# eboigne/PyTV-4D

Hardware: NVIDIA B200
Metric: cp_iter_voxel_updates_per_s (higher is better)
Workload: dtype f32

## Files before the change

__graft_entry__.py:

```python
import os
import subprocess
import sys
from concurrent.futures import ThreadPoolExecutor

ROOT = os.path.dirname(os.path.abspath(__file__))
CSRC = os.path.join(ROOT, "pytv-4d_b200", "csrc")
ARCH = ["-gencode", "arch=compute_100a,code=sm_100a"]
NVCC_FLAGS = ARCH + ["-lineinfo", "-O3", "-std=c++17", "-Xcompiler", "-fPIC"]
SOURCES = ["api.cu", "ops.cu", "tv.cu", "tv_tile.cu", "tv_tile_f64.cu", "tv_tile_norms.cu", "tv_tile_norms_f64.cu", "cp.cu", "cp_extra.cu", "cp_data.cu", "host_api.cu"]
HEADERS = ["core.cuh", "strip_core.cuh", "tile_core.cuh", "tile2_core.cuh", "kernels.cuh", "kernels2.cuh", "kernels_tile.cuh", "tv_path.cuh", "tv_args.cuh", "tmap.cuh", "tv_tile_impl.cuh", "host_common.cuh", os.path.join("..", "..", "include", "pytv_b200.h")]


def source_hash():
    import glob
    import hashlib
    files = sorted(os.path.basename(f) for f in glob.glob(os.path.join(CSRC, "*.cu")) + glob.glob(os.path.join(CSRC, "*.cuh")))
    h = hashlib.sha256()
    for f in files:
        h.update(open(os.path.join(CSRC, f), "rb").read())
    h.update(open(os.path.join(ROOT, "include", "pytv_b200.h"), "rb").read())
    return h.hexdigest()[:16]


def _stale(target, deps):
    if not os.path.exists(target):
        return True
    t = os.path.getmtime(target)
    return any(os.path.getmtime(d) > t for d in deps)


def build(force=False):
    os.makedirs(os.path.join(CSRC, "build"), exist_ok=True)
    hdrs = [os.path.join(CSRC, h) for h in HEADERS]
    src_hash = source_hash()

    def compile_one(src):
        obj = os.path.join(CSRC, "build", src.replace(".cu", ".o"))
        if force or _stale(obj, [os.path.join(CSRC, src)] + hdrs):
            subprocess.run(["nvcc"] + NVCC_FLAGS + ['-DPYTVB_SRC_HASH="%s"' % src_hash, "-c", src, "-o", obj], cwd=CSRC, check=True)
        return obj

    with ThreadPoolExecutor(max_workers=len(SOURCES)) as ex:
        objs = list(ex.map(compile_one, SOURCES))
    lib = os.path.join(CSRC, "libpytv_b200.so")
    if force or _stale(lib, objs):
        subprocess.run(["nvcc"] + ARCH + ["-shared", "-o", lib] + objs, cwd=CSRC, check=True)
    sys.path.insert(0, ROOT)
    if os.path.exists(os.path.join(ROOT, "tests", "emul_helper.py")):
        sys.path.insert(0, os.path.join(ROOT, "tests"))
        import emul_helper
        emul_helper.build_emul(force)
    import pytv_b200
    assert pytv_b200._lib.lib().pytvb_version() == 101
    assert pytv_b200._lib.lib().pytvb_build_id().decode() == src_hash, "the library on disk was not built from these sources"
    return lib


def smoke():
    sys.path.insert(0, ROOT)
    import numpy as np
    import torch
    import pytv_b200 as pytv
    from oracle import tv_oracle as orc

    assert torch.cuda.is_available(), "smoke() needs a CUDA device"
    torch.cuda.set_device(0)
    rs = np.random.RandomState(0)
    x = rs.rand(6, 3, 32, 32).astype(np.float32)
    kw = dict(reg_time=2 ** -5)
    for scheme in ("upwind", "downwind", "central", "hybrid"):
        tv, G = getattr(pytv.tv_GPU, "tv_" + scheme)(x.copy(), **kw)
        tv_o, G_o = orc.tv(x.astype(np.float64), scheme, **kw)
        assert abs(float(tv) - tv_o) <= 1e-5 * tv_o, (scheme, float(tv), tv_o)
        assert np.abs(G - G_o).max() <= 1e-5, (scheme, np.abs(G - G_o).max())
        Dx = getattr(pytv.tv_operators_GPU, "D_" + scheme)(x, **kw)
        assert np.abs(Dx - orc.D(x.astype(np.float64), scheme, **kw)).max() < 1e-5
        DTD = getattr(pytv.tv_operators_GPU, "D_T_" + scheme)(Dx, **kw)
        assert np.abs(DTD - orc.D_T(orc.D(x.astype(np.float64), scheme, **kw), scheme, **kw)).max() < 1e-5
    s = pytv.CPSolver(x, lam=0.1, scheme="hybrid", variant="rof", **kw)
    xo, xb, y = x.astype(np.float64), x.astype(np.float64), np.zeros((6, 8, 3, 32, 32))
    x0 = xo.copy()
    for _ in range(2):
        s.step()
        xo, xb, y, e = orc.cp_rof_step(xo, xb, x0, y, "hybrid", lam=0.1, sigma=0.5, tau=s.tau, theta=1.0, **kw)
    assert abs(s.energy() - e) <= 1e-5 * abs(e), (s.energy(), e)
    assert np.abs(s.result() - xo).max() < 1e-5
    print("smoke ok: TV/D/D_T/CP parity on cuda:0 (%s), %d kernel launches" % (torch.cuda.get_device_name(0), pytv._lib.lib().pytvb_launch_count()))


if __name__ == "__main__":
    build()
    if len(sys.argv) > 1 and sys.argv[1] == "smoke":
        smoke()
```

include/pytv_b200.h:

```cpp
#ifndef PYTV_B200_H
#define PYTV_B200_H

#include <stddef.h>
#include <stdint.h>

#ifdef __cplusplus
extern "C" {
#endif

#define PYTVB_VERSION 101

typedef enum { PYTVB_OK = 0, PYTVB_ERR_ARG = -1, PYTVB_ERR_CUDA = -2 } pytvb_status;

typedef enum { PYTVB_UPWIND = 0, PYTVB_DOWNWIND = 1, PYTVB_CENTRAL = 2, PYTVB_HYBRID = 3 } pytvb_scheme;
typedef enum { PYTVB_F32 = 0, PYTVB_F64 = 1 } pytvb_dtype;

typedef struct pytvb_problem {
    int32_t scheme;
    int32_t dtype;
    int64_t Nz, M, Ni, Nj;
    int64_t z_offset;
    int64_t Nz_global;
    double reg_z_over_reg;
    double reg_time;
    double factor_reg_static;
    const uint8_t* mask_static;
    const void* time_scale;
    const void* time_scale_lo;
    const void* time_scale_hi;
} pytvb_problem;

int pytvb_version(void);
const char* pytvb_build_id(void);
const char* pytvb_last_error(void);
uint64_t pytvb_launch_count(void);

int pytvb_num_components(const pytvb_problem* pb);

size_t pytvb_reduce_workspace_bytes(const pytvb_problem* pb);
size_t pytvb_tv_workspace_bytes(const pytvb_problem* pb);

int pytvb_D(const pytvb_problem* pb, const void* x, void* D, const void* halo_lo, const void* halo_hi, void* stream);

int pytvb_DT(const pytvb_problem* pb, const void* p, void* out, const void* halo_lo, const void* halo_hi, void* stream);

int pytvb_l21(const pytvb_problem* pb, const void* D, int64_t Nd, void* norms_or_null, double* d_sum, void* ws, void* stream);

int pytvb_apply_mask(const pytvb_problem* pb, void* x, const uint8_t* mask, int mask_is_plane, void* stream);

int pytvb_tv(const pytvb_problem* pb, const void* x, void* G, void* norms_or_null, double* d_tv, const void* halo_lo2,
             const void* halo_hi2, void* ws_reduce, void* ws_tv, void* stream);

int pytvb_gd_update(const pytvb_problem* pb, void* x, const void* x0, const void* G, double step, double lam, double* d_fid_or_null, void* ws,
                    void* stream);

int pytvb_tv_value(const pytvb_problem* pb, const void* x, double* d_tv, const void* halo_lo, const void* halo_hi, void* ws, void* stream);

int pytvb_cp_dual(const pytvb_problem* pb, const void* xbar, void* y, double lam, double sigma, double* d_l21_or_null,
                  const void* halo_lo, const void* halo_hi, void* ws, void* stream);

int pytvb_cp_primal_rof(const pytvb_problem* pb, const void* y, void* x, void* xbar, const void* x0, double tau, double theta,
                        double* d_fid_or_null, const void* halo_lo, const void* halo_hi, void* ws, void* stream);

int pytvb_cp_primal_readme(const pytvb_problem* pb, const void* y_tv, void* x, void* y_f, const void* x0, double tau,
                           double sigma_A, double* d_fid_or_null, const void* halo_lo, const void* halo_hi, void* ws,
                           void* stream);

int pytvb_cp_dual_p2p(const pytvb_problem* pb, const void* xbar, void* y, double lam, double sigma, double* d_l21_or_null,
                      const void* halo_lo, const void* halo_hi, void* mirror_prev, void* mirror_next, void* ws, void* stream);
int pytvb_cp_primal_p2p(const pytvb_problem* pb, int variant, const void* y, void* x, void* aux, const void* x0, double tau, double c2,
                        double* d_fid_or_null, const void* halo_lo, const void* halo_hi, void* mirror_prev, void* mirror_next, void* ws,
                        void* stream);

typedef enum { PYTVB_DATA_L2 = 0, PYTVB_DATA_L1 = 1 } pytvb_data_term;
int pytvb_cp_primal_data(const pytvb_problem* pb, int data_term, const void* data_weight, const void* y, void* x, void* xbar,
                         const void* x0, double tau, double theta, double* d_fid_or_null, const void* halo_lo, const void* halo_hi,
                         void* mirror_prev, void* mirror_next, void* ws, void* stream);

int pytvb_cp_dual_f16y(const pytvb_problem* pb, const void* xbar, void* y_half, double lam, double sigma, double* d_l21_or_null,
                       const void* halo_lo, const void* halo_hi, void* ws, void* stream);
int pytvb_cp_primal_rof_f16y(const pytvb_problem* pb, const void* y_half, void* x, void* xbar, const void* x0, double lam, double tau,
                             double theta, double* d_fid_or_null, const void* halo_lo_half, const void* halo_hi_half, void* ws, void* stream);

int pytvb_tv_host(const pytvb_problem* pb_host_mask , const void* x_host, void* G_host,
                  void* norms_host_or_null, double* tv_out);

typedef struct pytvb_cp_solver pytvb_cp_solver;
int pytvb_cp_create(const pytvb_problem* pb_host_mask, double lam, double sigma, double tau, double theta, pytvb_cp_solver** out);
int pytvb_cp_reset_host(pytvb_cp_solver* s, const void* x0_host);
int pytvb_cp_step_host(pytvb_cp_solver* s, const void* x0_host, void* x_host_or_null, double* energy_out);
int pytvb_cp_destroy(pytvb_cp_solver* s);

#ifdef __cplusplus
}
#endif
#endif
```

pytv-4d_b200/_lib.py:

```python
import ctypes
import os

_HERE = os.path.dirname(os.path.abspath(__file__))
LIB_PATH = os.environ.get("PYTVB_LIB_PATH") or os.path.join(_HERE, "csrc", "libpytv_b200.so")

SCHEME_ID = {"upwind": 0, "downwind": 1, "central": 2, "hybrid": 3}
F32, F64 = 0, 1


class Problem(ctypes.Structure):
    _fields_ = [
        ("scheme", ctypes.c_int32),
        ("dtype", ctypes.c_int32),
        ("Nz", ctypes.c_int64),
        ("M", ctypes.c_int64),
        ("Ni", ctypes.c_int64),
        ("Nj", ctypes.c_int64),
        ("z_offset", ctypes.c_int64),
        ("Nz_global", ctypes.c_int64),
        ("reg_z_over_reg", ctypes.c_double),
        ("reg_time", ctypes.c_double),
        ("factor_reg_static", ctypes.c_double),
        ("mask_static", ctypes.c_void_p),
        ("time_scale", ctypes.c_void_p),
        ("time_scale_lo", ctypes.c_void_p),
        ("time_scale_hi", ctypes.c_void_p),
    ]


def make_problem(scheme, dtype_id, shape, reg_z_over_reg=1.0, reg_time=0.0, factor_reg_static=0.0, mask_static_ptr=None,
                 z_offset=0, Nz_global=None, time_scale_ptr=None):
    Nz, M, Ni, Nj = (int(s) for s in shape)
    rz = float(reg_z_over_reg)
    return Problem(SCHEME_ID[scheme] if isinstance(scheme, str) else int(scheme), int(dtype_id), Nz, M, Ni, Nj, int(z_offset),
                   int(Nz if Nz_global is None else Nz_global), rz, float(reg_time), float(factor_reg_static),
                   ctypes.c_void_p(mask_static_ptr) if mask_static_ptr else None,
                   ctypes.c_void_p(time_scale_ptr) if time_scale_ptr else None, None, None)


_VP = ctypes.c_void_p
_PB = ctypes.POINTER(Problem)
_PROTOTYPES = {
    "pytvb_version": (ctypes.c_int, []),
    "pytvb_build_id": (ctypes.c_char_p, []),
    "pytvb_last_error": (ctypes.c_char_p, []),
    "pytvb_launch_count": (ctypes.c_uint64, []),
    "pytvb_num_components": (ctypes.c_int, [_PB]),
    "pytvb_reduce_workspace_bytes": (ctypes.c_size_t, [_PB]),
    "pytvb_tv_workspace_bytes": (ctypes.c_size_t, [_PB]),
    "pytvb_D": (ctypes.c_int, [_PB, _VP, _VP, _VP, _VP, _VP]),
    "pytvb_DT": (ctypes.c_int, [_PB, _VP, _VP, _VP, _VP, _VP]),
    "pytvb_l21": (ctypes.c_int, [_PB, _VP, ctypes.c_int64, _VP, _VP, _VP, _VP]),
    "pytvb_apply_mask": (ctypes.c_int, [_PB, _VP, _VP, ctypes.c_int, _VP]),
    "pytvb_tv": (ctypes.c_int, [_PB, _VP, _VP, _VP, _VP, _VP, _VP, _VP, _VP, _VP]),
    "pytvb_gd_update": (ctypes.c_int, [_PB, _VP, _VP, _VP, ctypes.c_double, ctypes.c_double, _VP, _VP, _VP]),
    "pytvb_tv_value": (ctypes.c_int, [_PB, _VP, _VP, _VP, _VP, _VP, _VP]),
    "pytvb_cp_dual": (ctypes.c_int, [_PB, _VP, _VP, ctypes.c_double, ctypes.c_double, _VP, _VP, _VP, _VP, _VP]),
    "pytvb_cp_primal_rof": (ctypes.c_int, [_PB, _VP, _VP, _VP, _VP, ctypes.c_double, ctypes.c_double, _VP, _VP, _VP, _VP, _VP]),
    "pytvb_cp_primal_readme": (ctypes.c_int, [_PB, _VP, _VP, _VP, _VP, ctypes.c_double, ctypes.c_double, _VP, _VP, _VP, _VP, _VP]),
    "pytvb_cp_dual_p2p": (ctypes.c_int, [_PB, _VP, _VP, ctypes.c_double, ctypes.c_double, _VP, _VP, _VP, _VP, _VP, _VP, _VP]),
    "pytvb_cp_primal_p2p": (ctypes.c_int, [_PB, ctypes.c_int, _VP, _VP, _VP, _VP, ctypes.c_double, ctypes.c_double, _VP, _VP, _VP, _VP, _VP, _VP, _VP]),
    "pytvb_cp_primal_data": (ctypes.c_int, [_PB, ctypes.c_int, _VP, _VP, _VP, _VP, _VP, ctypes.c_double, ctypes.c_double, _VP, _VP, _VP, _VP, _VP, _VP,
                                            _VP]),
    "pytvb_cp_dual_f16y": (ctypes.c_int, [_PB, _VP, _VP, ctypes.c_double, ctypes.c_double, _VP, _VP, _VP, _VP, _VP]),
    "pytvb_cp_primal_rof_f16y": (ctypes.c_int, [_PB, _VP, _VP, _VP, _VP, ctypes.c_double, ctypes.c_double, ctypes.c_double, _VP, _VP, _VP, _VP, _VP]),
    "pytvb_tv_host": (ctypes.c_int, [_PB, _VP, _VP, _VP, ctypes.POINTER(ctypes.c_double)]),
    "pytvb_cp_create": (ctypes.c_int, [_PB, ctypes.c_double, ctypes.c_double, ctypes.c_double, ctypes.c_double, ctypes.POINTER(_VP)]),
    "pytvb_cp_reset_host": (ctypes.c_int, [_VP, _VP]),
    "pytvb_cp_step_host": (ctypes.c_int, [_VP, _VP, _VP, ctypes.POINTER(ctypes.c_double)]),
    "pytvb_cp_destroy": (ctypes.c_int, [_VP]),
}

_lib = None


def lib():
    global _lib
    if _lib is None:
        if not os.path.exists(LIB_PATH):
            raise RuntimeError("pytv_b200: %s has not been built (run __graft_entry__.build()); there is no CPU fallback" % LIB_PATH)
        handle = ctypes.CDLL(LIB_PATH)
        for name, (res, args) in _PROTOTYPES.items():
            fn = getattr(handle, name)
            fn.restype = res
            fn.argtypes = args
        _lib = handle
    return _lib


class PytvError(RuntimeError):
    pass


def check(rc):
    if rc != 0:
        raise PytvError("pytv_b200 call failed (%d): %s" % (rc, lib().pytvb_last_error().decode("utf-8", "replace")))
```

pytv-4d_b200/cp.py:

```python
import ctypes
import os

import numpy as np
import torch

from . import _dev, _lib


DATA_TERMS = {"l2": 0, "l1": 1}


def partition_z(Nz_global, world_size):
    if Nz_global < world_size:
        raise ValueError("cannot split %d planes over %d ranks" % (Nz_global, world_size))
    base, rem = divmod(Nz_global, world_size)
    out, off = [], 0
    for r in range(world_size):
        n = base + (1 if r < rem else 0)
        out.append((off, n))
        off += n
    return out


def operator_norm_sq_bound(scheme, z_on, t_on, reg_z_over_reg, reg_time, factor_reg_static, has_mask_static, max_time_weight=1.0):
    w = 2.0
    if z_on:
        w += reg_z_over_reg
    if t_on:
        w += reg_time * (max(1.0, factor_reg_static) if has_mask_static else 1.0) * max(1.0, float(max_time_weight))
    return w if scheme == "central" else 4.0 * w


class CudaOps:

    def __init__(self):
        self.lib = _lib.lib()

    def cp_dual(self, pb, xbar, y, lam, sigma, d_l21, lo, hi, ws):
        if y.dtype == torch.float16:
            _lib.check(self.lib.pytvb_cp_dual_f16y(ctypes.byref(pb), _dev.ptr(xbar), _dev.ptr(y), lam, sigma, _dev.ptr(d_l21), _dev.ptr(lo),
                                                   _dev.ptr(hi), _dev.ptr(ws), _dev.stream_ptr()))
            return
        _lib.check(self.lib.pytvb_cp_dual(ctypes.byref(pb), _dev.ptr(xbar), _dev.ptr(y), lam, sigma, _dev.ptr(d_l21), _dev.ptr(lo), _dev.ptr(hi),
                                          _dev.ptr(ws), _dev.stream_ptr()))

    def cp_primal(self, variant, pb, y, x, aux, x0, tau, c2, d_fid, lo, hi, ws, lam=None):
        if y.dtype == torch.float16:
            _lib.check(self.lib.pytvb_cp_primal_rof_f16y(ctypes.byref(pb), _dev.ptr(y), _dev.ptr(x), _dev.ptr(aux), _dev.ptr(x0), lam, tau, c2,
                                                         _dev.ptr(d_fid), _dev.ptr(lo), _dev.ptr(hi), _dev.ptr(ws), _dev.stream_ptr()))
            return
        fn = self.lib.pytvb_cp_primal_rof if variant == "rof" else self.lib.pytvb_cp_primal_readme
        _lib.check(fn(ctypes.byref(pb), _dev.ptr(y), _dev.ptr(x), _dev.ptr(aux), _dev.ptr(x0), tau, c2, _dev.ptr(d_fid), _dev.ptr(lo), _dev.ptr(hi),
                      _dev.ptr(ws), _dev.stream_ptr()))

    def cp_primal_data(self, pb, data_term, w, y, x, xbar, x0, tau, theta, d_fid, lo, hi, mirror_prev, mirror_next, ws):
        _lib.check(self.lib.pytvb_cp_primal_data(ctypes.byref(pb), DATA_TERMS[data_term], _dev.ptr(w), _dev.ptr(y), _dev.ptr(x), _dev.ptr(xbar),
                                                 _dev.ptr(x0), tau, theta, _dev.ptr(d_fid), _dev.ptr(lo), _dev.ptr(hi), mirror_prev, mirror_next,
                                                 _dev.ptr(ws), _dev.stream_ptr()))

    def cp_dual_p2p(self, pb, xbar, y, lam, sigma, d_l21, lo, hi, mirror_prev, mirror_next, ws):
        _lib.check(self.lib.pytvb_cp_dual_p2p(ctypes.byref(pb), _dev.ptr(xbar), _dev.ptr(y), lam, sigma, _dev.ptr(d_l21), _dev.ptr(lo), _dev.ptr(hi),
                                              mirror_prev, mirror_next, _dev.ptr(ws), _dev.stream_ptr()))

    def cp_primal_p2p(self, variant, pb, y, x, aux, x0, tau, c2, d_fid, lo, hi, mirror_prev, mirror_next, ws):
        _lib.check(self.lib.pytvb_cp_primal_p2p(ctypes.byref(pb), 0 if variant == "rof" else 1, _dev.ptr(y), _dev.ptr(x), _dev.ptr(aux), _dev.ptr(x0),
                                                tau, c2, _dev.ptr(d_fid), _dev.ptr(lo), _dev.ptr(hi), mirror_prev, mirror_next, _dev.ptr(ws),
                                                _dev.stream_ptr()))

    def workspace(self, pb, device):
        return _dev.reduce_workspace(pb, device)

    def tv_value(self, pb, x, d_tv, lo, hi, ws):
        _lib.check(self.lib.pytvb_tv_value(ctypes.byref(pb), _dev.ptr(x), _dev.ptr(d_tv), _dev.ptr(lo), _dev.ptr(hi), _dev.ptr(ws), _dev.stream_ptr()))

    def adjoint(self, pb, y, out, lo, hi):
        _lib.check(self.lib.pytvb_DT(ctypes.byref(pb), _dev.ptr(y), _dev.ptr(out), _dev.ptr(lo), _dev.ptr(hi), _dev.stream_ptr()))


class HaloExchange:

    def __init__(self, group=None, reduce_group=None):
        import torch.distributed as dist
        self.dist = dist
        self.group = group
        self._reduce_group = reduce_group
        self.rank = dist.get_rank(group)
        self.world = dist.get_world_size(group)
        self.prev = self.rank - 1 if self.rank > 0 else None
        self.next = self.rank + 1 if self.rank < self.world - 1 else None

    def _global(self, r):
        return r if self.group is None else self.dist.get_global_rank(self.group, r)

    def exchange(self, to_prev, to_next, from_prev, from_next):
        self.finish(self.start_exchange(to_prev, to_next, from_prev, from_next))

    def finish(self, reqs):
        for req in reqs or ():
            req.wait()

    def start_exchange(self, to_prev, to_next, from_prev, from_next):
        ops = []
        P2P = self.dist.P2POp
        if self.prev is not None:
            if to_prev is not None:
                ops.append(P2P(self.dist.isend, to_prev, self._global(self.prev), self.group))
            if from_prev is not None:
                ops.append(P2P(self.dist.irecv, from_prev, self._global(self.prev), self.group))
        if self.next is not None:
            if to_next is not None:
                ops.append(P2P(self.dist.isend, to_next, self._global(self.next), self.group))
            if from_next is not None:
                ops.append(P2P(self.dist.irecv, from_next, self._global(self.next), self.group))
        return self.dist.batch_isend_irecv(ops) if ops else []

    def allreduce_sum(self, t):
        self.dist.all_reduce(t, op=self.dist.ReduceOp.SUM, group=self.group)
        return t

    def allreduce_sum_async(self, t):
        g = self._reduce_group if self._reduce_group is not None else self.group
        return self.dist.all_reduce(t, op=self.dist.ReduceOp.SUM, group=g, async_op=True)

    def make_reduce_group(self):
        if self._reduce_group is None and self.group is None:
            self._reduce_group = self.dist.new_group(ranks=list(range(self.dist.get_world_size())))


def neighbour_handshake(hdl, prev, nxt, timeout_ms, sync="auto"):
    if sync == "barrier" or not hasattr(hdl, "put_signal"):
        hdl.barrier(channel=0, timeout_ms=timeout_ms)
        return
    if nxt is not None:
        hdl.put_signal(nxt, channel=1, timeout_ms=timeout_ms)
    if prev is not None:
        hdl.put_signal(prev, channel=2, timeout_ms=timeout_ms)
    if prev is not None:
        hdl.wait_signal(prev, channel=1, timeout_ms=timeout_ms)
    if nxt is not None:
        hdl.wait_signal(nxt, channel=2, timeout_ms=timeout_ms)


class PeerHalos:
    IMG_LO, IMG_HI, FLD_LO, FLD_HI = 0, 1, 2, 3

    def __init__(self, halo, plane, dtype, device):
        import torch.distributed._symmetric_memory as symm
        group = halo.group if halo.group is not None else halo.dist.group.WORLD
        self.buf = symm.empty((4,) + tuple(plane), dtype=dtype, device=device)
        self.hdl = symm.rendezvous(self.buf, group)
        self.buf.zero_()
        self.plane_bytes = self.buf[0].numel() * self.buf.element_size()
        self.timeout_ms = int(os.environ.get("PYTVB_P2P_TIMEOUT_MS", "60000"))
        self.sync = os.environ.get("PYTVB_P2P_SYNC", "auto")
        self.prev, self.next = halo.prev, halo.next
        self.hdl.barrier(channel=0, timeout_ms=self.timeout_ms)

    def local(self, slot):
        return self.buf[slot]

    def peer(self, rank, slot):
        return None if rank is None else int(self.hdl.buffer_ptrs[rank]) + slot * self.plane_bytes

    def barrier(self):
        neighbour_handshake(self.hdl, self.prev, self.next, self.timeout_ms, self.sync)


class CPSolver:

    def __init__(self, x0, lam, scheme="hybrid", variant="rof", sigma=0.5, tau=None, theta=1.0, sigma_A=1.0, reg_z_over_reg=1.0,
                 reg_time=0.0, mask_static=False, factor_reg_static=0, distributed=False, group=None, z_offset=None, Nz_global=None,
                 ops=None, track_energy=True, dual_dtype=None, time_weight=None, comm=None, reduce_group=None, data_term="l2", data_weight=None):
        if scheme not in _dev.SCHEMES:
            raise ValueError("unknown scheme %r" % (scheme,))
        if variant not in ("rof", "readme"):
            raise ValueError("variant must be 'rof' or 'readme'")
        if data_term not in DATA_TERMS:
            raise ValueError("data_term must be 'l2' or 'l1'")
        self.ops = ops if ops is not None else CudaOps()
        self.scheme, self.variant = scheme, variant
        self.lam, self.sigma, self.theta, self.sigma_A = float(lam), float(sigma), float(theta), float(sigma_A)
        self.track_energy = track_energy
        shape = _dev.image_shape(x0)
        if ops is None:
            self.x0, _ = _dev.to_device(x0)
            if self.x0.data_ptr() == (x0.data_ptr() if isinstance(x0, torch.Tensor) else 0):
                self.x0 = self.x0.clone()
        else:
            self.x0 = torch.as_tensor(np.ascontiguousarray(x0)).clone() if not isinstance(x0, torch.Tensor) else x0.clone().contiguous()
        dev, dt = self.x0.device, self.x0.dtype
        self.halo = HaloExchange(group, reduce_group) if (distributed or group is not None) else None
        if self.halo is not None and self.halo.world > 1:
            if track_energy:
                self.halo.make_reduce_group()
            if (Nz_global is None) != (z_offset is None):
                raise ValueError("sharded solver: give both z_offset and Nz_global, or neither (they are then derived from the ranks' plane counts)")
            if Nz_global is None:
                counts = torch.zeros(self.halo.world, dtype=torch.int64, device=dev)
                counts[self.halo.rank] = shape[0]
                self.halo.allreduce_sum(counts)
                Nz_global = int(counts.sum().item())
                z_offset = int(counts[: self.halo.rank].sum().item())
        else:
            self.halo = None
        self.z_offset = int(z_offset or 0)
        self.Nz_global = int(Nz_global if Nz_global is not None else shape[0])
        self.shape = shape
        self._ms = None
        if not isinstance(mask_static, bool):
            if ops is None:
                self._ms = _dev.mask_static_to_device(mask_static, shape[2], shape[3])
            else:
                m = mask_static if isinstance(mask_static, torch.Tensor) else torch.as_tensor(np.asarray(mask_static))
                self._ms = (m.reshape(shape[2], shape[3]) != 0).to(torch.uint8).contiguous()
        self._ts = None
        max_tw = 1.0
        if time_weight is not None:
            w = time_weight if isinstance(time_weight, torch.Tensor) else torch.as_tensor(np.asarray(time_weight))
            w = torch.broadcast_to(w.to(dev).to(torch.float64), shape)
            if bool((w < 0).any()):
                raise ValueError("time_weight must be >= 0")
            self._ts = torch.sqrt(w).to(dt).contiguous()
            mx = w.max().reshape(1).clone()
            if self.halo is not None:
                self.halo.dist.all_reduce(mx, op=self.halo.dist.ReduceOp.MAX, group=self.halo.group)
            max_tw = float(mx.item())
        self.data_term = data_term
        self._dw = None
        self._w_min = 1.0
        if data_weight is not None:
            w = data_weight if isinstance(data_weight, torch.Tensor) else torch.as_tensor(np.asarray(data_weight))
            w = torch.broadcast_to(w.to(dev).to(torch.float64), shape)
            if not bool(torch.isfinite(w).all()) or bool((w < 0).any()):
                raise ValueError("data_weight must be finite and >= 0")
            self._dw = w.to(dt).contiguous()
            mn = self._dw.min().double().reshape(1).clone()
            if self.halo is not None:
                self.halo.dist.all_reduce(mn, op=self.halo.dist.ReduceOp.MIN, group=self.halo.group)
            self._w_min = float(mn.item())
        self._data = data_term != "l2" or self._dw is not None
        self.pb = _lib.make_problem(scheme, _lib.F32 if dt == torch.float32 else _lib.F64, shape, float(reg_z_over_reg), float(reg_time),
                                    float(factor_reg_static), self._ms.data_ptr() if self._ms is not None else None, self.z_offset,
                                    self.Nz_global, self._ts.data_ptr() if self._ts is not None else None)
        self.z_on = self.Nz_global > 1 and float(reg_z_over_reg) > 0
        self.t_on = shape[1] > 1 and float(reg_time) > 0
        self.Nd = (4 + 2 * self.z_on + 2 * self.t_on) if scheme == "hybrid" else (2 + self.z_on + self.t_on)
        if tau is None:
            L2 = operator_norm_sq_bound(scheme, self.z_on, self.t_on, float(reg_z_over_reg), float(reg_time), float(factor_reg_static),
                                        self._ms is not None, max_tw)
            tau = 1.0 / (L2 + 1.0)
        self.tau = float(tau)
        self.x = self.x0.clone()
        self.aux = self.x0.clone() if variant == "rof" else torch.zeros_like(self.x0)
        self.dual_dtype = dt if dual_dtype is None else dual_dtype
        if self.dual_dtype != dt:
            if self.dual_dtype != torch.float16 or dt != torch.float32 or variant != "rof":
                raise ValueError("dual_dtype=torch.float16 needs float32 images and variant='rof'")
            if not self.lam > 0:
                raise ValueError("half-precision dual storage needs lam > 0")
        if self._data and (variant != "rof" or self.dual_dtype != dt):
            raise ValueError("data_term='l1' and data_weight need variant='rof' and full-precision duals")
        self.y = torch.zeros((shape[0], self.Nd) + shape[1:], dtype=self.dual_dtype, device=dev)
        self.scal = torch.zeros(6, dtype=torch.float64, device=dev)
        self.overlap = os.environ.get("PYTVB_OVERLAP", "0") == "1"
        self._pending = None
        self._field_req = None
        self._pb_cache = {}
        self.ws = self.ops.workspace(self.pb, dev)
        self.iterations = 0
        self._img_lo = self._img_hi = self._fld_lo = self._fld_hi = None
        self._peer = None
        if comm is None:
            comm = os.environ.get("PYTVB_COMM", "auto")
        if comm not in ("auto", "nccl", "p2p"):
            raise ValueError("comm must be 'auto', 'nccl' or 'p2p'")
        if self.halo is not None and self.z_on:
            plane = (shape[1], shape[2], shape[3])
            interior_lo, interior_hi = self.halo.prev is not None, self.halo.next is not None
            need_img_lo, need_img_hi = scheme != "upwind", scheme != "downwind"
            need_fld_lo, need_fld_hi = scheme != "downwind", scheme != "upwind"
            p2p_ok = (ops is None and self.dual_dtype == dt and not self.overlap
                      and str(self.halo.dist.get_backend(self.halo.group)).lower() == "nccl")
            if comm == "p2p" and not p2p_ok:
                raise ValueError("comm='p2p' needs the CUDA executor over an NCCL group, the blocking schedule and full-precision duals")
            if comm != "nccl" and p2p_ok:
                try:
                    self._peer = PeerHalos(self.halo, plane, dt, dev)
                except Exception as exc:
                    if comm == "p2p":
                        raise
                    self._peer_error = repr(exc)
                if comm == "auto":
                    ok = torch.tensor([1 if self._peer is not None else 0], dtype=torch.int32, device=dev)
                    self.halo.dist.all_reduce(ok, op=self.halo.dist.ReduceOp.MIN, group=self.halo.group)
                    if int(ok.item()) == 0:
                        self._peer = None
            if self._peer is not None:
                mk = lambda d=dt, slot=0: self._peer.local(slot)
            else:
                mk = lambda d=dt, slot=0: torch.empty(plane, dtype=d, device=dev)
            self._img_lo = mk(slot=0) if (interior_lo and need_img_lo) else None
            self._img_hi = mk(slot=1) if (interior_hi and need_img_hi) else None
            self._fld_lo = mk(self.dual_dtype, 2) if (interior_lo and need_fld_lo) else None
            self._fld_hi = mk(self.dual_dtype, 3) if (interior_hi and need_fld_hi) else None
            if self._peer is not None:
                P, h = self._peer, self.halo
                self._mir_A = (P.peer(h.prev, P.FLD_HI) if need_fld_hi else None, P.peer(h.next, P.FLD_LO) if need_fld_lo else None)
                self._mir_B = (P.peer(h.prev, P.IMG_HI) if need_img_hi else None, P.peer(h.next, P.IMG_LO) if need_img_lo else None)
        self._zf = 4 if scheme == "hybrid" else 2
        self._zb = 5 if scheme == "hybrid" else 2

    def _dual_input(self):
        return self.aux if self.variant == "rof" else self.x

    def _image_planes(self):
        src = self._dual_input()
        return (src[0] if self.scheme != "downwind" else None, src[-1] if self.scheme != "upwind" else None)

    def _start_image_exchange(self):
        return self.halo.start_exchange(*self._image_planes(), self._img_lo, self._img_hi)

    def _start_field_exchange(self):
        to_prev = self.y[0, self._zb] if self.scheme != "upwind" else None
        to_next = self.y[-1, self._zf] if self.scheme != "downwind" else None
        return self.halo.start_exchange(to_prev, to_next, self._fld_lo, self._fld_hi)

    def _sub_problem(self, a, b):
        key = (a, b)
        pb = self._pb_cache.get(key)
        if pb is None:
            pb = _lib.Problem.from_buffer_copy(self.pb)
            pb.Nz = b - a
            pb.z_offset = self.z_offset + a
            if self._ts is not None:
                pb.time_scale = self._ts[a].data_ptr()
            self._pb_cache[key] = pb
        return pb

    def _dual_range(self, a, b, slot):
        if b <= a:
            return
        u = self._dual_input()
        Nz = self.shape[0]
        lo = u[a - 1] if a > 0 else self._img_lo
        hi = u[b] if b < Nz else self._img_hi
        d = self.scal[slot:slot + 1] if self.track_energy else None
        self.ops.cp_dual(self._sub_problem(a, b), u[a:b], self.y[a:b], self.lam, self.sigma, d, lo, hi, self.ws)

    def _primal_range(self, a, b, slot):
        if b <= a:
            return
        Nz = self.shape[0]
        lo = self.y[a - 1, self._zf] if a > 0 else self._fld_lo
        hi = self.y[b, self._zb] if b < Nz else self._fld_hi
        d = self.scal[3 + slot:4 + slot] if self.track_energy else None
        if self._data:
            self.ops.cp_primal_data(self._sub_problem(a, b), self.data_term, self._dw[a:b] if self._dw is not None else None, self.y[a:b], self.x[a:b],
                                    self.aux[a:b], self.x0[a:b], self.tau, self.theta, d, lo, hi, None, None, self.ws)
            return
        c2 = self.theta if self.variant == "rof" else self.sigma_A
        if self.y.dtype == torch.float16:
            self.ops.cp_primal(self.variant, self._sub_problem(a, b), self.y[a:b], self.x[a:b], self.aux[a:b], self.x0[a:b], self.tau, c2, d, lo, hi,
                               self.ws, lam=self.lam)
        else:
            self.ops.cp_primal(self.variant, self._sub_problem(a, b), self.y[a:b], self.x[a:b], self.aux[a:b], self.x0[a:b], self.tau, c2, d, lo,
                               hi, self.ws)

    def _split(self):
        return self.halo is not None and self.z_on and self.overlap and self.shape[0] >= 2

    def _pass_A(self):
        Nz = self.shape[0]
        if self.halo is None or not self.z_on:
            self._dual_range(0, Nz, 0)
            return
        if self._peer is None:
            if self._pending is None:
                self._pending = self._start_image_exchange()
            self.halo.finish(self._pending)
            self._pending = None
        if self.track_energy:
            self.scal[0:3].zero_()
        if self._peer is not None:
            if self._pending is None:
                self.halo.exchange(*self._image_planes(), self._img_lo, self._img_hi)
                self._peer.barrier()
            self._pending = ()
            d = self.scal[0:1] if self.track_energy else None
            self.ops.cp_dual_p2p(self.pb, self._dual_input(), self.y, self.lam, self.sigma, d, self._img_lo, self._img_hi, self._mir_A[0],
                                 self._mir_A[1], self.ws)
            self._peer.barrier()
            self._field_req = ()
            return
        if not self._split():
            self._dual_range(0, Nz, 0)
            self._field_req = self._start_field_exchange()
            return
        self._dual_range(0, 1, 0)
        self._dual_range(Nz - 1, Nz, 1)
        self._field_req = self._start_field_exchange()
        self._dual_range(1, Nz - 1, 2)

    def _pass_B(self):
        Nz = self.shape[0]
        if self.halo is None or not self.z_on:
            self._primal_range(0, Nz, 0)
            return
        self.halo.finish(self._field_req)
        self._field_req = None
        if self.track_energy:
            self.scal[3:6].zero_()
        if self._peer is not None:
            d = self.scal[3:4] if self.track_energy else None
            if self._data:
                self.ops.cp_primal_data(self.pb, self.data_term, self._dw, self.y, self.x, self.aux, self.x0, self.tau, self.theta, d, self._fld_lo,
                                        self._fld_hi, self._mir_B[0], self._mir_B[1], self.ws)
            else:
                c2 = self.theta if self.variant == "rof" else self.sigma_A
                self.ops.cp_primal_p2p(self.variant, self.pb, self.y, self.x, self.aux, self.x0, self.tau, c2, d, self._fld_lo, self._fld_hi,
                                       self._mir_B[0], self._mir_B[1], self.ws)
            self._peer.barrier()
            self._pending = ()
            return
        if not self._split():
            self._primal_range(0, Nz, 0)
            self._pending = self._start_image_exchange()
            return
        self._primal_range(0, 1, 0)
        self._primal_range(Nz - 1, Nz, 1)
        self._pending = self._start_image_exchange()
        self._primal_range(1, Nz - 1, 2)

    def capture_graph(self, iterations=1):
        if self.halo is not None:
            raise RuntimeError("capture_graph is not supported for distributed solvers")
        self._graph = None
        torch.cuda.synchronize()
        state = (self.x.clone(), self.aux.clone(), self.y.clone(), self.scal.clone(), self.iterations)
        side = torch.cuda.Stream()
        side.wait_stream(torch.cuda.current_stream())
        with torch.cuda.stream(side):
            self.step(1)
        torch.cuda.current_stream().wait_stream(side)
        g = torch.cuda.CUDAGraph()
        with torch.cuda.graph(g):
            self.step(iterations)
        self.x.copy_(state[0]); self.aux.copy_(state[1]); self.y.copy_(state[2]); self.scal.copy_(state[3])
        self.iterations = state[4]
        self._graph, self._graph_iters = g, int(iterations)
        self._graph_key = self._graph_state_key()
        return self

    def _graph_state_key(self):
        return (self.x0.data_ptr(), self.x.data_ptr(), self.aux.data_ptr(), self.y.data_ptr(), self.lam, self.sigma, self.tau, self.theta, self.sigma_A,
                self._dw.data_ptr() if self._dw is not None else 0)

    def step(self, n=1):
        g = getattr(self, "_graph", None)
        if g is not None and self._graph_key != self._graph_state_key():
            g = self._graph = None
        if g is not None and not torch.cuda.is_current_stream_capturing():
            while n >= self._graph_iters:
                g.replay()
                self.iterations += self._graph_iters
                n -= self._graph_iters
        for _ in range(n):
            self._pass_A()
            self._pass_B()
            self.iterations += 1
        return self

    def step_host(self, x0_host, x_out_host=None):
        src = x0_host if isinstance(x0_host, torch.Tensor) else torch.from_numpy(x0_host)
        self.x0.copy_(src, non_blocking=True)
        self.step(1)
        if x_out_host is not None:
            dst = x_out_host if isinstance(x_out_host, torch.Tensor) else torch.from_numpy(x_out_host)
            dst.copy_(self.x, non_blocking=True)
        return self.energy()

    PIPE_DEPTH = 3

    def _pipe_init(self):
        if getattr(self, "_pipe", None) is None:
            dev = self.x0.device
            D = self.PIPE_DEPTH
            self._pipe = dict(
                h2d=torch.cuda.Stream(device=dev), d2h=torch.cuda.Stream(device=dev),
                x0=[self.x0] + [torch.empty_like(self.x0) for _ in range(D - 1)],
                snap=[torch.empty_like(self.x) for _ in range(D)],
                scal=[torch.zeros(6, dtype=torch.float64, device=dev) for _ in range(D)],
                scal_host=[torch.zeros(6, dtype=torch.float64).pin_memory() for _ in range(D)],
                d2h_done=[None] * D, comp_done=[None] * D, k=0)
        return self._pipe

    def step_host_async(self, x0_host, x_out_host=None):
        p = self._pipe_init()
        k = p["k"]
        slot = k % self.PIPE_DEPTH
        cur = torch.cuda.current_stream()
        src = x0_host if isinstance(x0_host, torch.Tensor) else torch.from_numpy(x0_host)
        if p["comp_done"][slot] is not None:
            p["h2d"].wait_event(p["comp_done"][slot])
        else:
            first = torch.cuda.Event()
            first.record(cur)
            p["h2d"].wait_event(first)
        with torch.cuda.stream(p["h2d"]):
            p["x0"][slot].copy_(src, non_blocking=True)
            up = torch.cuda.Event()
            up.record()
        cur.wait_event(up)
        self.x0 = p["x0"][slot]
        self.step(1)
        if p["d2h_done"][slot] is not None:
            cur.wait_event(p["d2h_done"][slot])
        p["snap"][slot].copy_(self.x)
        p["scal"][slot].copy_(self.scal)
        done = torch.cuda.Event()
        done.record()
        p["comp_done"][slot] = done
        p["d2h"].wait_event(done)
        with torch.cuda.stream(p["d2h"]):
            if x_out_host is not None:
                dst = x_out_host if isinstance(x_out_host, torch.Tensor) else torch.from_numpy(x_out_host)
                dst.copy_(p["snap"][slot], non_blocking=True)
            p["scal_host"][slot].copy_(p["scal"][slot], non_blocking=True)
            ev = torch.cuda.Event()
            ev.record()
        p["d2h_done"][slot] = ev
        p["k"] = k + 1
        return (k, slot, ev)

    def wait(self, ticket):
        k, slot, ev = ticket
        ev.synchronize()
        h = self._pipe["scal_host"][slot]
        s = torch.stack((h[0:3].sum(), h[3:6].sum()))
        if self.halo is not None:
            s = s.to(self.x0.device)
            self.halo.allreduce_sum(s)
        return self._energy_of(*s.tolist())

    def _energy_of(self, l21, fid):
        return (0.5 * fid if self.data_term == "l2" else fid) + self.lam * l21

    def energy_async(self):
        if not self.track_energy:
            raise RuntimeError("energy tracking was disabled")
        s = torch.stack((self.scal[0:3].sum(), self.scal[3:6].sum()))
        work = self.halo.allreduce_sum_async(s) if self.halo is not None else None
        return (s, work)

    def energy_result(self, handle):
        s, work = handle
        if work is not None:
            work.wait()
        return self._energy_of(*s.tolist())

    def energy(self):
        if not self.track_energy:
            raise RuntimeError("energy tracking was disabled")
        s = torch.stack((self.scal[0:3].sum(), self.scal[3:6].sum()))
        if self.halo is not None:
            self.halo.allreduce_sum(s)
        return self._energy_of(*s.tolist())

    def _sync_halos_for_diagnostics(self):
        if self.halo is not None and self._pending is not None:
            self.halo.finish(self._pending)
            self._pending = None

    def primal_energy(self):
        lo = hi = None
        if self.halo is not None and self.z_on:
            self._sync_halos_for_diagnostics()
            to_prev = self.x[0] if self.scheme != "downwind" else None
            to_next = self.x[-1] if self.scheme != "upwind" else None
            self.halo.exchange(to_prev, to_next, self._img_lo, self._img_hi)
            lo, hi = self._img_lo, self._img_hi
        d = torch.zeros(2, dtype=torch.float64, device=self.x.device)
        self.ops.tv_value(self.pb, self.x, d[0:1], lo, hi, self.ws)
        if not self._data:
            d[1] = torch.sum((self.x - self.x0).double() ** 2) if self.x.numel() < (1 << 28) else sum(
                torch.sum((self.x[k] - self.x0[k]).double() ** 2) for k in range(self.shape[0]))
        else:
            for k in range(self.shape[0]):
                r = (self.x[k] - self.x0[k]).double()
                r = r * r if self.data_term == "l2" else r.abs()
                d[1] += torch.sum(r * self._dw[k].double() if self._dw is not None else r)
        if self.halo is not None:
            self.halo.allreduce_sum(d)
        tv, fid = d.tolist()
        return self._energy_of(tv, fid)

    def dual_energy(self):
        if self._data and not self._w_min > 0:
            raise ValueError("the dual energy is unbounded where data_weight = 0: no duality gap (solve() uses the energy change)")
        lo = hi = None
        if self.halo is not None and self.z_on:
            to_prev = self.y[0, self._zb] if self.scheme != "upwind" else None
            to_next = self.y[-1, self._zf] if self.scheme != "downwind" else None
            self.halo.exchange(to_prev, to_next, self._fld_lo, self._fld_hi)
            lo, hi = self._fld_lo, self._fld_hi
        dty = torch.empty_like(self.x)
        if self.y.dtype != self.x.dtype:
            raise NotImplementedError("the duality gap is not available with half-precision dual storage")
        self.ops.adjoint(self.pb, self.y, dty, lo, hi)
        if self._data:
            return self._dual_energy_data(dty)
        d = torch.zeros(2, dtype=torch.float64, device=self.x.device)
        for k in range(self.shape[0]):
            x0k = self.x0[k].double()
            d[0] += torch.sum(x0k * x0k)
            d[1] += torch.sum((x0k - dty[k].double()) ** 2)
        if self.halo is not None:
            self.halo.allreduce_sum(d)
        a, b = d.tolist()
        return 0.5 * a - 0.5 * b

    def _dual_energy_data(self, dty):
        d = torch.zeros(2, dtype=torch.float64, device=self.x.device)
        for k in range(self.shape[0]):
            s, x0k = dty[k].double(), self.x0[k].double()
            w = self._dw[k].double() if self._dw is not None else None
            if self.data_term == "l2":
                d[0] += torch.sum(s * x0k - s * s / (2.0 * w))
            else:
                d[0] += torch.sum(s * x0k)
                d[1] = torch.maximum(d[1], (s.abs() / w if w is not None else s.abs()).max())
        if self.halo is not None:
            self.halo.allreduce_sum(d[0:1])
            self.halo.dist.all_reduce(d[1:2], op=self.halo.dist.ReduceOp.MAX, group=self.halo.group)
        a, m = d.tolist()
        if self.data_term == "l2":
            return a
        return a * (1.0 / m if m > 1.0 else 1.0)

    def gap(self):
        p, d = self.primal_energy(), self.dual_energy()
        return p, d, p - d

    def solve(self, max_iter=1000, tol=1e-4, check_every=25, callback=None):
        if self._data and not self._w_min > 0:
            return self._solve_by_energy(max_iter, tol, check_every, callback)
        info = dict(iterations=0, converged=False, criterion="gap")
        it = 0
        while it < max_iter:
            n = min(check_every, max_iter - it)
            self.step(n)
            it += n
            p, d, g = self.gap()
            if callback is not None:
                callback(self, it, p, d)
            info.update(iterations=it, primal=p, dual=d, gap=g, relative_gap=g / max(abs(p), 1e-300))
            if g <= tol * max(abs(p), 1e-300):
                info["converged"] = True
                break
        return info

    def _solve_by_energy(self, max_iter, tol, check_every, callback):
        info = dict(iterations=0, converged=False, criterion="energy")
        it, p_prev = 0, None
        while it < max_iter:
            n = min(check_every, max_iter - it)
            self.step(n)
            it += n
            p = self.primal_energy()
            if callback is not None:
                callback(self, it, p, None)
            info.update(iterations=it, primal=p)
            if p_prev is not None:
                info["relative_change"] = abs(p - p_prev) / max(abs(p), 1e-300)
                if info["relative_change"] <= tol:
                    info["converged"] = True
                    break
            p_prev = p
        return info

    def set_data(self, x0, reset_primal=False, reset_dual=False):
        src = x0 if isinstance(x0, torch.Tensor) else torch.as_tensor(np.ascontiguousarray(x0))
        self.x0.copy_(src.to(self.x0.dtype), non_blocking=True)
        if reset_primal:
            self.x.copy_(self.x0)
            if self.variant == "rof":
                self.aux.copy_(self.x0)
            self._pending = None
        if reset_dual:
            self.y.zero_()
        return self

    def result(self, return_pytorch_tensor=False):
        return self.x if return_pytorch_tensor else self.x.detach().cpu().numpy()


class TVProx:

    def __init__(self, example, lam, scheme="hybrid", n_iter=20, **weights):
        self.solver = CPSolver(example, lam, scheme=scheme, variant="rof", track_energy=False, **weights)
        self.n_iter = int(n_iter)

    def __call__(self, v, lam=None, n_iter=None):
        if lam is not None:
            self.solver.lam = float(lam)
        self.solver.set_data(v, reset_primal=True)
        self.solver.step(self.n_iter if n_iter is None else int(n_iter))
        return self.solver.x


def denoise_tv_chambolle(image, weight=0.1, eps=2e-4, max_num_iter=200, channel_axis=None):
    img = np.asarray(image) if not isinstance(image, torch.Tensor) else image
    was_tensor = isinstance(img, torch.Tensor)
    arr = img if was_tensor else torch.as_tensor(np.ascontiguousarray(img))
    if channel_axis is not None:
        arr = arr.movedim(channel_axis, 0)
        spatial = arr.shape[1:]
        vol = arr.reshape((arr.shape[0],) + tuple(spatial))
        vol = vol[None] if len(spatial) == 2 else vol.movedim(0, 1)
    else:
        spatial = arr.shape
        vol = arr.reshape((1, 1) + tuple(spatial)) if len(spatial) == 2 else arr.reshape((spatial[0], 1) + tuple(spatial[1:]))
    if len(spatial) not in (2, 3):
        raise ValueError("denoise_tv_chambolle handles 2-D and 3-D images")
    vol = vol.contiguous()
    if vol.dtype not in (torch.float32, torch.float64):
        vol = vol.to(torch.float64)
    solver = CPSolver(vol, weight, scheme="upwind", variant="rof", reg_z_over_reg=1.0, reg_time=0.0)
    e_prev = e_init = None
    for it in range(int(max_num_iter)):
        solver.step(1)
        e = solver.energy()
        if it == 0:
            e_init = e
        elif abs(e_prev - e) < eps * e_init:
            break
        e_prev = e
    out = solver.x
    if channel_axis is not None:
        out = out[0] if len(spatial) == 2 else out.movedim(1, 0)
        out = out.movedim(0, channel_axis)
    else:
        out = out.reshape(tuple(spatial))
    return out if was_tensor else out.cpu().numpy()


def gd_denoise(x0, lam, n_iter, step, scheme="hybrid", return_pytorch_tensor=False, return_losses=False, graph=None, reg_z_over_reg=1.0,
               reg_time=0.0, mask_static=False, factor_reg_static=0, time_weight=None):
    x0d, was_tensor = _dev.to_device(x0)
    if x0d.data_ptr() == (x0.data_ptr() if isinstance(x0, torch.Tensor) else 0):
        x0d = x0d.clone()
    shape = _dev.image_shape(x0d)
    lib = _lib.lib()
    n_iter = int(n_iter)
    ms = _dev.mask_static_to_device(mask_static, shape[2], shape[3])
    ts = _dev.time_scale_to_device(time_weight, shape, x0d)
    pb = _dev.problem(scheme, x0d, shape, reg_z_over_reg, reg_time, factor_reg_static, ms, ts=ts)
    x = x0d.clone()
    G = torch.empty_like(x)
    ws_r = _dev.reduce_workspace(pb, x.device)
    ws_t = torch.empty(lib.pytvb_tv_workspace_bytes(ctypes.byref(pb)), dtype=torch.uint8, device=x.device)
    tvs = torch.zeros(max(n_iter, 1), dtype=torch.float64, device=x.device)
    fids = torch.zeros(max(n_iter, 1), dtype=torch.float64, device=x.device)

    def iteration(it):
        st = _dev.stream_ptr()
        _lib.check(lib.pytvb_tv(ctypes.byref(pb), _dev.ptr(x), _dev.ptr(G), None, _dev.ptr(tvs[it:it + 1]), None, None, _dev.ptr(ws_r), _dev.ptr(ws_t), st))
        _lib.check(lib.pytvb_gd_update(ctypes.byref(pb), _dev.ptr(x), _dev.ptr(x0d), _dev.ptr(G), float(step), float(lam),
                                       _dev.ptr(fids[it:it + 1]) if return_losses else None, _dev.ptr(ws_r), st))

    if graph is None:
        graph = x.numel() < (1 << 22) and n_iter >= 8
    if graph and n_iter > 0:
        torch.cuda.synchronize()
        side = torch.cuda.Stream()
        side.wait_stream(torch.cuda.current_stream())
        with torch.cuda.stream(side):
            iteration(0)
        torch.cuda.current_stream().wait_stream(side)
        x.copy_(x0d)
        g = torch.cuda.CUDAGraph()
        with torch.cuda.graph(g):
            for it in range(n_iter):
                iteration(it)
        g.replay()
    else:
        for it in range(n_iter):
            iteration(it)
    out = x if (return_pytorch_tensor or was_tensor) else x.cpu().numpy()
    if return_losses:
        return out, (0.5 * fids[:n_iter] + float(lam) * tvs[:n_iter]).cpu().numpy()
    return out


def cp_denoise(x0, lam, n_iter, scheme="hybrid", variant="rof", return_pytorch_tensor=False, return_energy=False, **kw):
    solver = CPSolver(x0, lam, scheme=scheme, variant=variant, track_energy=return_energy, **kw)
    solver.step(int(n_iter))
    if isinstance(x0, torch.Tensor):
        return_pytorch_tensor = True
    out = solver.result(return_pytorch_tensor)
    return (out, solver.energy()) if return_energy else out
```

pytv-4d_b200/csrc/strip_core.cuh:

```cuda
#pragma once
#include <cuda_fp16.h>

#include "core.cuh"

namespace pytvb {

PYTVB_HD float fast_rsqrt(float a) {
#if defined(__CUDA_ARCH__)
    return rsqrtf(a);
#else
    return 1.0f / sqrtf(a);
#endif
}
PYTVB_HD double fast_rsqrt(double a) { return 1.0 / sqrt(a); }
PYTVB_HD float fast_sqrt(float a) {
#if defined(__CUDA_ARCH__)
    float r;
    asm("sqrt.approx.f32 %0, %1;" : "=f"(r) : "f"(a));
    return r;
#else
    return sqrtf(a);
#endif
}
PYTVB_HD double fast_sqrt(double a) { return sqrt(a); }

template <typename T, typename YT, int VEC>
PYTVB_HD void ld_y(T* dst, const YT* src) {
    const Pack<YT, VEC> p = ld_pack<YT, VEC>(src);
#pragma unroll
    for (int e = 0; e < VEC; ++e) dst[e] = (T)p.v[e];
}
template <typename T, typename YT, int VEC>
PYTVB_HD void st_y(YT* dst, const T* v) {
    Pack<YT, VEC> p;
#pragma unroll
    for (int e = 0; e < VEC; ++e) p.v[e] = (YT)v[e];
    st_pack<YT, VEC>(dst, p);
}

template <typename T, int VEC>
PYTVB_HD void st_pack_stream(T* p, const Pack<T, VEC>& v) {
#if defined(__CUDA_ARCH__)
    if constexpr (sizeof(T) == 4 && VEC == 4) { __stcs(reinterpret_cast<float4*>(p), *reinterpret_cast<const float4*>(&v)); return; }
    if constexpr (sizeof(T) == 8 && VEC == 2) { __stcs(reinterpret_cast<double2*>(p), *reinterpret_cast<const double2*>(&v)); return; }
#endif
    st_pack<T, VEC>(p, v);
}

template <typename T, typename YT = T>
struct DualPlane {
    const T* c;
    const T* zm; const T* zp;
    const T* tm; const T* tp;
    YT* y;
    T fz, ft;
    const T* ts;
};

template <typename T, int SCHEME, typename YT = T>
PYTVB_HD DualPlane<T, YT> make_dual_plane(const ImgView<T>& X, YT* y, const Params<T>& P, int z, int t) {
    DualPlane<T, YT> d;
    const long long zg = P.zg0 + z;
    const bool v_zm = zg > 0, v_zp = zg < P.NzG - 1, v_tm = t > 0, v_tp = t < P.M - 1;
    d.c = X.row(P, z, t, 0);
    d.zm = v_zm ? X.row(P, z - 1, t, 0) : d.c;
    d.zp = v_zp ? X.row(P, z + 1, t, 0) : d.c;
    d.tm = v_tm ? X.row(P, z, t - 1, 0) : d.c;
    d.tp = v_tp ? X.row(P, z, t + 1, 0) : d.c;
    d.y = y + (long long)z * P.sZf + (long long)t * P.sT;
    d.fz = d.ft = T(1);
    d.ts = (P.tscale && z >= 0 && z < P.Nz) ? P.tscale + (long long)z * P.sZ + (long long)t * P.sT : nullptr;
    if (SCHEME == CENTRAL) {
        if (P.z_fwd_fallback) d.zm = d.c; else d.fz = (v_zm && v_zp) ? T(1) : T(0);
        if (P.t_fwd_fallback) d.tm = d.c; else d.ft = (v_tm && v_tp) ? T(1) : T(0);
    }
    return d;
}

template <typename T, int VEC>
PYTVB_HD void time_factor(T* f, const Params<T>& P, const T* ts_plane, int i, int j0, int o) {
    static_factor<T, VEC>(f, P, i, j0);
    if (ts_plane) {
        const Pack<T, VEC> sc = ld_pack<T, VEC>(ts_plane + o);
#pragma unroll
        for (int e = 0; e < VEC; ++e) f[e] *= sc.v[e];
    }
}
template <typename T, int VEC>
PYTVB_HD void scale_by(T* v, const T* ts_plane, int o) {
    if (ts_plane) {
        const Pack<T, VEC> sc = ld_pack<T, VEC>(ts_plane + o);
#pragma unroll
        for (int e = 0; e < VEC; ++e) v[e] *= sc.v[e];
    }
}

template <typename T, int VEC, int SCHEME, bool Z_ON, bool T_ON, typename YT, bool TS>
PYTVB_HD void strip_raw_diffs_impl(T (*d)[VEC], const DualPlane<T, YT>& pl, const Params<T>& P, int i, int j0, int o, int o_up, int o_dn) {
    typedef Comp<SCHEME, Z_ON, T_ON> C;
    T c[VEC + 2], up[VEC], dn[VEC], zm[VEC], zp[VEC], tm[VEC], tp[VEC];
    ld_into<T, VEC>(c + 1, pl.c + o);
    c[0] = (C::NEED_BWD && j0 > 0) ? pl.c[o - 1] : c[1];
    c[VEC + 1] = (C::NEED_FWD && j0 + VEC < P.Nj) ? pl.c[o + VEC] : c[VEC];
    if (C::NEED_BWD) ld_into<T, VEC>(up, pl.c + o_up);
    if (C::NEED_FWD) ld_into<T, VEC>(dn, pl.c + o_dn);
    if (Z_ON && C::NEED_BWD) ld_into<T, VEC>(zm, pl.zm + o);
    if (Z_ON && C::NEED_FWD) ld_into<T, VEC>(zp, pl.zp + o);
    if (T_ON && C::NEED_BWD) ld_into<T, VEC>(tm, pl.tm + o);
    if (T_ON && C::NEED_FWD) ld_into<T, VEC>(tp, pl.tp + o);
    T fac[VEC];
    if (T_ON) { if constexpr (TS) time_factor<T, VEC>(fac, P, pl.ts, i, j0, o); else static_factor<T, VEC>(fac, P, i, j0); }
    const T fi = (SCHEME == CENTRAL) ? ((i > 0 && i < P.Ni - 1) ? T(1) : T(0)) : T(1);
#pragma unroll
    for (int e = 0; e < VEC; ++e) {
        const T x = c[e + 1];
        if (SCHEME == HYBRID) {
            d[C::I_F][e] = dn[e] - x;
            d[C::J_F][e] = c[e + 2] - x;
            d[C::I_B][e] = x - up[e];
            d[C::J_B][e] = x - c[e];
            if (Z_ON) { d[C::Z_F][e] = P.srz * (zp[e] - x); d[C::Z_B][e] = P.srz * (x - zm[e]); }
            if (T_ON) { const T w = P.srt * fac[e]; d[C::T_F][e] = w * (tp[e] - x); d[C::T_B][e] = w * (x - tm[e]); }
        } else if (SCHEME == UPWIND) {
            d[0][e] = dn[e] - x;
            d[1][e] = c[e + 2] - x;
            if (Z_ON) d[C::Z_F][e] = P.srz * (zp[e] - x);
            if (T_ON) d[C::T_F][e] = P.srt * fac[e] * (tp[e] - x);
        } else if (SCHEME == DOWNWIND) {
            d[0][e] = x - up[e];
            d[1][e] = x - c[e];
            if (Z_ON) d[C::Z_F][e] = P.srz * (x - zm[e]);
            if (T_ON) d[C::T_F][e] = P.srt * fac[e] * (x - tm[e]);
        } else {
            const int j = j0 + e;
            const T fj = (j > 0 && j < P.Nj - 1) ? T(1) : T(0);
            d[0][e] = fi * (dn[e] - up[e]);
            d[1][e] = fj * (c[e + 2] - c[e]);
            if (Z_ON) d[C::Z_F][e] = (P.srz * pl.fz) * (zp[e] - zm[e]);
            if (T_ON) d[C::T_F][e] = (P.srt * pl.ft * fac[e]) * (tp[e] - tm[e]);
        }
    }
}

template <typename T, int VEC, int SCHEME, bool Z_ON, bool T_ON, typename YT = T, bool TS = false>
PYTVB_HD void strip_raw_diffs(T (*d)[VEC], const DualPlane<T, YT>& pl, const Params<T>& P, int i, int j0, int o, int o_up, int o_dn) {
    strip_raw_diffs_impl<T, VEC, SCHEME, Z_ON, T_ON, YT, TS && T_ON>(d, pl, P, i, j0, o, o_up, o_dn);
}

template <typename YT>
struct MirrorPlanes {
    YT* prev;
    YT* next;
};

template <typename YT>
struct MirrorBufs {
    YT* prev;
    YT* next;
};
template <typename YT, typename PT>
PYTVB_HD MirrorPlanes<YT> mirror_planes(const MirrorBufs<YT>& m, const PT& P, int z, int t) {
    MirrorPlanes<YT> r;
    r.prev = (m.prev && z == 0) ? m.prev + (long long)t * P.sT : nullptr;
    r.next = (m.next && z == P.Nz - 1) ? m.next + (long long)t * P.sT : nullptr;
    return r;
}
template <typename T, int VEC, int SCHEME, bool Z_ON, bool T_ON, typename YT = T, bool TS = false, bool MIR = false>
PYTVB_HD T strip_quad_cp_dual(const DualPlane<T, YT>& pl, const Params<T>& P, int i, int j0, int o, int o_up, int o_dn, T sig, T lam,
                              MirrorPlanes<YT> mir = MirrorPlanes<YT>{nullptr, nullptr}) {
    typedef Comp<SCHEME, Z_ON, T_ON> C;
    constexpr int ND = C::ND;
    T y[ND][VEC], d[ND][VEC];
#pragma unroll
    for (int k = 0; k < ND; ++k) ld_y<T, YT, VEC>(y[k], pl.y + (long long)k * P.sC + o);
    strip_raw_diffs<T, VEC, SCHEME, Z_ON, T_ON, YT, TS>(d, pl, P, i, j0, o, o_up, o_dn);
    T l21 = T(0);
#pragma unroll
    for (int e = 0; e < VEC; ++e) {
        T s = T(0), sd = T(0);
#pragma unroll
        for (int k = 0; k < ND; ++k) {
            sd += d[k][e] * d[k][e];
            y[k][e] += sig * d[k][e];
            s += y[k][e] * y[k][e];
        }
        l21 += fast_sqrt(sd);
        const T r = lam * fast_rsqrt(s);
        const T scale = r < T(1) ? r : T(1);
#pragma unroll
        for (int k = 0; k < ND; ++k) y[k][e] *= scale;
    }
#pragma unroll
#pragma unroll
    for (int k = 0; k < ND; ++k) st_y<T, YT, VEC>(pl.y + (long long)k * P.sC + o, y[k]);
    if constexpr (MIR && Z_ON) {
        if (mir.prev) st_y<T, YT, VEC>(mir.prev + o, y[C::Z_B]);
        if (mir.next) st_y<T, YT, VEC>(mir.next + o, y[C::Z_F]);
    }
    return l21;
}

template <typename T, int VEC, int SCHEME, bool Z_ON, bool T_ON, bool TS = false>
PYTVB_HD void strip_quad_D(T* out, const DualPlane<T>& pl, const Params<T>& P, int i, int j0, int o, int o_up, int o_dn) {
    typedef Comp<SCHEME, Z_ON, T_ON> C;
    T d[C::ND][VEC];
    strip_raw_diffs<T, VEC, SCHEME, Z_ON, T_ON, T, TS>(d, pl, P, i, j0, o, o_up, o_dn);
#pragma unroll
    for (int k = 0; k < C::ND; ++k) {
        Pack<T, VEC> pk;
#pragma unroll
        for (int e = 0; e < VEC; ++e) pk.v[e] = d[k][e] * P.inv_div;
        st_pack_stream<T, VEC>(out + (long long)k * P.sC + o, pk);
    }
}

template <typename T, int VEC, int SCHEME, bool Z_ON, bool T_ON, bool TS = false>
PYTVB_HD T strip_quad_tv_norm(T* w_plane, T* n_plane, const DualPlane<T>& pl, const Params<T>& P, int i, int j0, int o, int o_up, int o_dn) {
    typedef Comp<SCHEME, Z_ON, T_ON> C;
    T d[C::ND][VEC];
    strip_raw_diffs<T, VEC, SCHEME, Z_ON, T_ON, T, TS>(d, pl, P, i, j0, o, o_up, o_dn);
    Pack<T, VEC> w, n;
    T sum = T(0);
#pragma unroll
    for (int e = 0; e < VEC; ++e) {
        T s = T(0);
#pragma unroll
        for (int k = 0; k < C::ND; ++k) s += d[k][e] * d[k][e];
        const T rs = fast_rsqrt(s);
        const T nr = s > T(0) ? s * rs * P.inv_div : T(0);
        w.v[e] = s > T(0) ? rs * P.div : T(0);
        n.v[e] = s > T(0) ? nr : T(INFINITY);
        sum += nr;
    }
    if (w_plane) st_pack<T, VEC>(w_plane + o, w);
    if (n_plane) st_pack<T, VEC>(n_plane + o, n);
    return sum;
}

template <typename T, typename YT = T>
struct PrimalPlane {
    const YT* y;
    const YT* zf_m;
    const YT* zb_p;
    const YT* tf_m;
    const YT* tb_p;
    T az, bz, at, bt;
    long long img;
    const T* ts_m; const T* ts_c; const T* ts_p;
};

template <typename T, int SCHEME>
PYTVB_HD void adj_factors(T& a, T& b, long long k, long long L, bool fallback) {
    if (SCHEME == CENTRAL && !fallback) {
        a = (k >= 2) ? T(1) : T(0);
        b = (k <= L - 3) ? T(1) : T(0);
    } else {
        a = (k > 0) ? T(1) : T(0);
        b = (k < L - 1) ? T(1) : T(0);
    }
}

template <typename T, int SCHEME, bool Z_ON, bool T_ON, typename YT = T>
PYTVB_HD PrimalPlane<T, YT> make_primal_plane(const FieldView<YT>& Y, const Params<T>& P, int z, int t) {
    typedef Comp<SCHEME, Z_ON, T_ON> C;
    PrimalPlane<T, YT> p;
    p.y = Y.row(P, z, 0, t, 0);
    p.img = (long long)z * P.sZ + (long long)t * P.sT;
    p.zf_m = p.zb_p = p.tf_m = p.tb_p = p.y;
    p.az = p.bz = p.at = p.bt = T(0);
    p.ts_m = p.ts_c = p.ts_p = nullptr;
    if (T_ON && P.tscale) {
        p.ts_c = P.tscale + p.img;
        p.ts_m = t > 0 ? p.ts_c - P.sT : p.ts_c;
        p.ts_p = t < P.M - 1 ? p.ts_c + P.sT : p.ts_c;
    }
    if (Z_ON) {
        const long long zg = P.zg0 + z;
        T a, b;
        adj_factors<T, SCHEME>(a, b, zg, P.NzG, P.z_fwd_fallback != 0);
        p.az = a * P.srz;
        p.bz = b * P.srz;
        if (zg > 0) p.zf_m = Y.row(P, z - 1, C::Z_F, t, 0);
        if (zg < P.NzG - 1) p.zb_p = Y.row(P, z + 1, C::Z_B, t, 0);
    }
    if (T_ON) {
        T a, b;
        adj_factors<T, SCHEME>(a, b, t, P.M, P.t_fwd_fallback != 0);
        p.at = a * P.srt;
        p.bt = b * P.srt;
        if (t > 0) p.tf_m = Y.row(P, z, C::T_F, t - 1, 0);
        if (t < P.M - 1) p.tb_p = Y.row(P, z, C::T_B, t + 1, 0);
    }
    return p;
}

template <typename T, int SCHEME>
PYTVB_HD void adj_operands(T& m, T& p, T f_m, T f_c, T b_c, T b_p, bool fallback) {
    if (SCHEME == UPWIND || (SCHEME == CENTRAL && fallback)) { m = f_m; p = f_c; }
    else if (SCHEME == DOWNWIND) { m = b_c; p = b_p; }
    else if (SCHEME == HYBRID) { m = f_m + b_c; p = f_c + b_p; }
    else { m = f_m; p = b_p; }
}

template <typename T, int VEC> struct CgLoad;
#if defined(__CUDACC__)
template <> struct CgLoad<float, 4> { static __device__ __forceinline__ void ld(float* d, const float* p) { const float4 v = __ldcg(reinterpret_cast<const float4*>(p)); d[0] = v.x; d[1] = v.y; d[2] = v.z; d[3] = v.w; } };
template <> struct CgLoad<float, 1> { static __device__ __forceinline__ void ld(float* d, const float* p) { d[0] = __ldcg(p); } };
template <> struct CgLoad<double, 2> { static __device__ __forceinline__ void ld(double* d, const double* p) { const double2 v = __ldcg(reinterpret_cast<const double2*>(p)); d[0] = v.x; d[1] = v.y; } };
template <> struct CgLoad<double, 1> { static __device__ __forceinline__ void ld(double* d, const double* p) { d[0] = __ldcg(p); } };
#endif
template <typename T, int VEC, bool CG, typename YT>
PYTVB_HD void ld_field(T* dst, const YT* src) {
#if defined(__CUDA_ARCH__)
    if constexpr (CG) { CgLoad<T, VEC>::ld(dst, (const T*)src); return; }
#endif
    ld_y<T, YT, VEC>(dst, src);
}
template <typename T, bool CG, typename YT>
PYTVB_HD T ld_field1(const YT* src) {
#if defined(__CUDA_ARCH__)
    if constexpr (CG) { T v; CgLoad<T, 1>::ld(&v, (const T*)src); return v; }
#endif
    T v;
    ld_y<T, YT, 1>(&v, src);
    return v;
}

template <typename T, int VEC, int SCHEME, bool Z_ON, bool T_ON, bool CG, typename YT, bool TS>
PYTVB_HD void strip_quad_DT_impl(T* out, const PrimalPlane<T, YT>& pl, const Params<T>& P, int i, int j0, int o, int o_up, int o_dn) {
    typedef Comp<SCHEME, Z_ON, T_ON> C;
    constexpr bool NF = (SCHEME != DOWNWIND);
    constexpr bool NB = (SCHEME != UPWIND);
    constexpr bool CTR = (SCHEME == CENTRAL);
    const YT* yI_F = pl.y + (long long)C::I_F * P.sC;
    const YT* yI_B = pl.y + (long long)C::I_B * P.sC;
    const YT* yJ_F = pl.y + (long long)C::J_F * P.sC;
    const YT* yJ_B = pl.y + (long long)C::J_B * P.sC;
    T acc[VEC];
    {
        T a, b, f_m[VEC], f_c[VEC], b_c[VEC], b_p[VEC];
        adj_factors<T, SCHEME>(a, b, i, P.Ni, false);
        if (NF) ld_field<T, VEC, CG>(f_m, yI_F + o_up); else zero_into<T, VEC>(f_m);
        if (!CTR && NF) ld_field<T, VEC, CG>(f_c, yI_F + o); else zero_into<T, VEC>(f_c);
        if (!CTR && NB) ld_field<T, VEC, CG>(b_c, yI_B + o); else zero_into<T, VEC>(b_c);
        if (NB) ld_field<T, VEC, CG>(b_p, yI_B + o_dn); else zero_into<T, VEC>(b_p);
#pragma unroll
        for (int e = 0; e < VEC; ++e) {
            T m, p;
            adj_operands<T, SCHEME>(m, p, f_m[e], f_c[e], b_c[e], b_p[e], false);
            acc[e] = a * m - b * p;
        }
    }
    {
        T f[VEC + 2], bq[VEC + 2];
#pragma unroll
        for (int e = 0; e < VEC + 2; ++e) bq[e] = T(0);
        ld_field<T, VEC, CG>(f + 1, yJ_F + o);
        f[0] = (NF && j0 > 0) ? ld_field1<T, CG>(yJ_F + o - 1) : T(0);
        f[VEC + 1] = (CTR && j0 + VEC < P.Nj) ? ld_field1<T, CG>(yJ_F + o + VEC) : T(0);
        if (SCHEME == HYBRID || SCHEME == DOWNWIND) {
            if (SCHEME == HYBRID) ld_field<T, VEC, CG>(bq + 1, yJ_B + o);
            else {
#pragma unroll
                for (int e = 0; e < VEC + 2; ++e) bq[e] = f[e];
            }
            bq[VEC + 1] = (j0 + VEC < P.Nj) ? ld_field1<T, CG>(yJ_B + o + VEC) : T(0);
        }
#pragma unroll
        for (int e = 0; e < VEC; ++e) {
            const int j = j0 + e;
            T a, b, m, p;
            adj_factors<T, SCHEME>(a, b, j, P.Nj, false);
            if (CTR) adj_operands<T, SCHEME>(m, p, f[e], T(0), T(0), f[e + 2], false);
            else adj_operands<T, SCHEME>(m, p, f[e], f[e + 1], bq[e + 1], bq[e + 2], false);
            acc[e] += a * m - b * p;
        }
    }
    if (Z_ON) {
        const bool fb = P.z_fwd_fallback != 0;
        const bool up_form = !CTR || fb;
        T f_m[VEC], f_c[VEC], b_c[VEC], b_p[VEC];
        if (NF) ld_field<T, VEC, CG>(f_m, pl.zf_m + o); else zero_into<T, VEC>(f_m);
        if (up_form && NF) ld_field<T, VEC, CG>(f_c, pl.y + (long long)C::Z_F * P.sC + o); else zero_into<T, VEC>(f_c);
        if (!CTR && NB) ld_field<T, VEC, CG>(b_c, pl.y + (long long)C::Z_B * P.sC + o); else zero_into<T, VEC>(b_c);
        if (NB && !(CTR && fb)) ld_field<T, VEC, CG>(b_p, pl.zb_p + o); else zero_into<T, VEC>(b_p);
#pragma unroll
        for (int e = 0; e < VEC; ++e) {
            T m, p;
            adj_operands<T, SCHEME>(m, p, f_m[e], f_c[e], b_c[e], b_p[e], fb);
            acc[e] += pl.az * m - pl.bz * p;
        }
    }
    if (T_ON) {
        const bool fb = P.t_fwd_fallback != 0;
        const bool up_form = !CTR || fb;
        T f_m[VEC], f_c[VEC], b_c[VEC], b_p[VEC], fac[VEC];
        if (NF) ld_field<T, VEC, CG>(f_m, pl.tf_m + o); else zero_into<T, VEC>(f_m);
        if (up_form && NF) ld_field<T, VEC, CG>(f_c, pl.y + (long long)C::T_F * P.sC + o); else zero_into<T, VEC>(f_c);
        if (!CTR && NB) ld_field<T, VEC, CG>(b_c, pl.y + (long long)C::T_B * P.sC + o); else zero_into<T, VEC>(b_c);
        if (NB && !(CTR && fb)) ld_field<T, VEC, CG>(b_p, pl.tb_p + o); else zero_into<T, VEC>(b_p);
        if constexpr (TS) {
            scale_by<T, VEC>(f_m, pl.ts_m, o); scale_by<T, VEC>(f_c, pl.ts_c, o);
            scale_by<T, VEC>(b_c, pl.ts_c, o); scale_by<T, VEC>(b_p, pl.ts_p, o);
        }
        static_factor<T, VEC>(fac, P, i, j0);
#pragma unroll
        for (int e = 0; e < VEC; ++e) {
            T m, p;
            adj_operands<T, SCHEME>(m, p, f_m[e], f_c[e], b_c[e], b_p[e], fb);
            acc[e] += (pl.at * m - pl.bt * p) * fac[e];
        }
    }
#pragma unroll
    for (int e = 0; e < VEC; ++e) out[e] = acc[e] * P.inv_div;
}

template <typename T, int VEC, int SCHEME, bool Z_ON, bool T_ON, bool CG = false, typename YT = T, bool TS = false>
PYTVB_HD void strip_quad_DT(T* out, const PrimalPlane<T, YT>& pl, const Params<T>& P, int i, int j0, int o, int o_up, int o_dn) {
    strip_quad_DT_impl<T, VEC, SCHEME, Z_ON, T_ON, CG, YT, TS && T_ON>(out, pl, P, i, j0, o, o_up, o_dn);
}

template <typename T, int VEC, int SCHEME, bool Z_ON, bool T_ON, int VARIANT, bool CG = false, typename YT = T, bool TS = false, bool MIR = false,
          bool WM = false>
PYTVB_HD T strip_quad_cp_primal(T* x, T* aux, const T* x0, const PrimalPlane<T, YT>& pl, const Params<T>& P, int i, int j0, int o, int o_up, int o_dn,
                                T tau, T c1, T c2, T tau_x0 = T(-1), MirrorPlanes<T> mir = MirrorPlanes<T>{nullptr, nullptr}, const T* wgt = nullptr) {
    T dty[VEC];
    strip_quad_DT<T, VEC, SCHEME, Z_ON, T_ON, CG, YT, TS>(dty, pl, P, i, j0, o, o_up, o_dn);
    if (tau_x0 < T(0)) tau_x0 = tau;
    const long long off = pl.img + o;
    const Pack<T, VEC> xo = ld_pack<T, VEC>(x + off), x0q = ld_pack<T, VEC>(x0 + off);
    Pack<T, VEC> xn, ax;
    T fid = T(0);
    if constexpr (VARIANT == 0) {
#pragma unroll
        for (int e = 0; e < VEC; ++e) {
            xn.v[e] = (xo.v[e] - tau * dty[e] + tau_x0 * x0q.v[e]) * c1;
            ax.v[e] = xn.v[e] + c2 * (xn.v[e] - xo.v[e]);
            const T r = xn.v[e] - x0q.v[e];
            fid += r * r;
        }
    } else if constexpr (VARIANT == 1) {
        const Pack<T, VEC> yf = ld_pack<T, VEC>(aux + off);
#pragma unroll
        for (int e = 0; e < VEC; ++e) {
            ax.v[e] = (yf.v[e] + c2 * (xo.v[e] - x0q.v[e])) * c1;
            xn.v[e] = xo.v[e] - tau * ax.v[e] - tau * dty[e];
            const T r = xn.v[e] - x0q.v[e];
            fid += r * r;
        }
    } else {
        static_assert(VARIANT == 2 || VARIANT == 3, "unknown primal variant");
        Pack<T, VEC> wq;
        if constexpr (WM) wq = ld_pack<T, VEC>(wgt + off);
#pragma unroll
        for (int e = 0; e < VEC; ++e) {
            T w = T(1), tw = tau_x0;
            if constexpr (WM) { w = wq.v[e]; tw = tau_x0 * w; }
            const T v = xo.v[e] - tau * dty[e];
            T r;
            if constexpr (VARIANT == 2) {
                xn.v[e] = (v + tw * x0q.v[e]) / (T(1) + tw);
                r = xn.v[e] - x0q.v[e];
                fid += w * (r * r);
            } else {
                const T d = v - x0q.v[e];
                const T a = (d < T(0) ? -d : d) - tw;
                const T s = a > T(0) ? a : T(0);
                xn.v[e] = x0q.v[e] + (d < T(0) ? -s : s);
                r = xn.v[e] - x0q.v[e];
                fid += w * (r < T(0) ? -r : r);
            }
            ax.v[e] = xn.v[e] + c2 * (xn.v[e] - xo.v[e]);
        }
    }
    st_pack<T, VEC>(x + off, xn);
    st_pack<T, VEC>(aux + off, ax);
    if constexpr (MIR && Z_ON) {
        const Pack<T, VEC>& u = (VARIANT == 1) ? xn : ax;
        if (mir.prev) st_pack<T, VEC>(mir.prev + o, u);
        if (mir.next) st_pack<T, VEC>(mir.next + o, u);
    }
    return fid;
}

template <typename T>
struct GradPlane {
    const T* x;  const T* xzm;  const T* xzp;  const T* xtm;  const T* xtp;
    const T* xzm2; const T* xzp2; const T* xtm2; const T* xtp2;
    const T* w;  const T* wzm;  const T* wzp;  const T* wtm;  const T* wtp;
    T az, bz, at, bt;
    bool z_fb, t_fb;
    const T* ts_m; const T* ts_c; const T* ts_p;
};

template <typename T, int SCHEME>
PYTVB_HD GradPlane<T> make_grad_plane(const ImgView<T>& X, const ImgView<T>& W, const Params<T>& P, int z, int t) {
    GradPlane<T> g;
    const long long zg = P.zg0 + z;
    const bool v_zm = zg > 0, v_zp = zg < P.NzG - 1, v_tm = t > 0, v_tp = t < P.M - 1;
    g.x = X.row(P, z, t, 0);
    g.w = W.row(P, z, t, 0);
    g.xzm = v_zm ? X.row(P, z - 1, t, 0) : g.x;  g.wzm = v_zm ? W.row(P, z - 1, t, 0) : g.w;
    g.xzp = v_zp ? X.row(P, z + 1, t, 0) : g.x;  g.wzp = v_zp ? W.row(P, z + 1, t, 0) : g.w;
    g.xtm = v_tm ? X.row(P, z, t - 1, 0) : g.x;  g.wtm = v_tm ? W.row(P, z, t - 1, 0) : g.w;
    g.xtp = v_tp ? X.row(P, z, t + 1, 0) : g.x;  g.wtp = v_tp ? W.row(P, z, t + 1, 0) : g.w;
    g.xzm2 = g.xzp2 = g.xtm2 = g.xtp2 = g.x;
    g.az = g.bz = P.srz;
    g.at = g.bt = P.srt;
    g.z_fb = P.z_fwd_fallback != 0;
    g.t_fb = P.t_fwd_fallback != 0;
    g.ts_m = g.ts_c = g.ts_p = nullptr;
    if (P.tscale) {
        g.ts_c = P.tscale + (long long)z * P.sZ + (long long)t * P.sT;
        g.ts_m = v_tm ? g.ts_c - P.sT : g.ts_c;
        g.ts_p = v_tp ? g.ts_c + P.sT : g.ts_c;
    }
    if (SCHEME == CENTRAL) {
        if (!g.z_fb) {
            if (zg >= 2) g.xzm2 = X.row(P, z - 2, t, 0); else g.az = T(0);
            if (zg <= P.NzG - 3) g.xzp2 = X.row(P, z + 2, t, 0); else g.bz = T(0);
        }
        if (!g.t_fb) {
            if (t >= 2) g.xtm2 = X.row(P, z, t - 2, 0); else g.at = T(0);
            if (t <= P.M - 3) g.xtp2 = X.row(P, z, t + 2, 0); else g.bt = T(0);
        }
    }
    return g;
}

template <typename T, int SCHEME>
PYTVB_HD T strip_g_axis(bool fallback, T a, T b, T xm2, T xm, T xc, T xp, T xp2, T wm, T wc, T wp) {
    if (SCHEME == UPWIND || (SCHEME == CENTRAL && fallback)) return (xc - xm) * wm - (xp - xc) * wc;
    if (SCHEME == DOWNWIND) return (xc - xm) * wc - (xp - xc) * wp;
    if (SCHEME == HYBRID) return (xc - xm) * (wm + wc) - (xp - xc) * (wc + wp);
    return a * ((xc - xm2) * wm) - b * ((xp2 - xc) * wp);
}

template <typename T, int VEC, int SCHEME, bool Z_ON, bool T_ON, bool TS, bool ROWS = true>
PYTVB_HD void strip_quad_G_impl(T* g_plane, const GradPlane<T>& pl, const Params<T>& P, int i, int j0, int o, const T* g_rows = nullptr) {
    constexpr bool CEN = (SCHEME == CENTRAL);
    const int Nj = P.Nj;
    const int o_up = i > 0 ? o - Nj : o, o_dn = i < P.Ni - 1 ? o + Nj : o;
    T xr[VEC + 4], wr[VEC + 2];
    ld_into<T, VEC>(xr + 2, pl.x + o);
    ld_into<T, VEC>(wr + 1, pl.w + o);
    xr[1] = j0 > 0 ? pl.x[o - 1] : xr[2];
    wr[0] = j0 > 0 ? pl.w[o - 1] : wr[1];
    xr[VEC + 2] = j0 + VEC < Nj ? pl.x[o + VEC] : xr[VEC + 1];
    wr[VEC + 1] = j0 + VEC < Nj ? pl.w[o + VEC] : wr[VEC];
    xr[0] = (CEN && j0 > 1) ? pl.x[o - 2] : xr[1];
    xr[VEC + 3] = (CEN && j0 + VEC + 1 < Nj) ? pl.x[o + VEC + 1] : xr[VEC + 2];
    T g[VEC];
#pragma unroll
    for (int e = 0; e < VEC; ++e) {
        const int j = j0 + e;
        const T a = (CEN && j < 2) ? T(0) : T(1), b = (CEN && j > Nj - 3) ? T(0) : T(1);
        g[e] = strip_g_axis<T, SCHEME>(false, a, b, xr[e], xr[e + 1], xr[e + 2], xr[e + 3], xr[e + 4], wr[e], wr[e + 1], wr[e + 2]);
    }
    if constexpr (ROWS) {
        T xm[VEC], xp[VEC], wm[VEC], wp[VEC], xm2[VEC], xp2[VEC];
        ld_into<T, VEC>(xm, pl.x + o_up);  ld_into<T, VEC>(xp, pl.x + o_dn);
        ld_into<T, VEC>(wm, pl.w + o_up);  ld_into<T, VEC>(wp, pl.w + o_dn);
        T a = T(1), b = T(1);
        if (CEN) {
            ld_into<T, VEC>(xm2, pl.x + (i > 1 ? o - 2 * Nj : o));
            ld_into<T, VEC>(xp2, pl.x + (i < P.Ni - 2 ? o + 2 * Nj : o));
            a = i >= 2 ? T(1) : T(0);
            b = i <= P.Ni - 3 ? T(1) : T(0);
        }
#pragma unroll
        for (int e = 0; e < VEC; ++e)
            g[e] += strip_g_axis<T, SCHEME>(false, a, b, CEN ? xm2[e] : T(0), xm[e], xr[e + 2], xp[e], CEN ? xp2[e] : T(0), wm[e], wr[e + 1], wp[e]);
    } else {
#pragma unroll
        for (int e = 0; e < VEC; ++e) g[e] += g_rows[e];
    }
    if (Z_ON) {
        T xm[VEC], xp[VEC], wm[VEC], wp[VEC], xm2[VEC], xp2[VEC];
        ld_into<T, VEC>(xm, pl.xzm + o);  ld_into<T, VEC>(xp, pl.xzp + o);
        ld_into<T, VEC>(wm, pl.wzm + o);  ld_into<T, VEC>(wp, pl.wzp + o);
        if (CEN) { ld_into<T, VEC>(xm2, pl.xzm2 + o); ld_into<T, VEC>(xp2, pl.xzp2 + o); }
#pragma unroll
        for (int e = 0; e < VEC; ++e) {
            const T v = strip_g_axis<T, SCHEME>(pl.z_fb, pl.az, pl.bz, CEN ? xm2[e] : T(0), xm[e], xr[e + 2], xp[e], CEN ? xp2[e] : T(0), wm[e], wr[e + 1], wp[e]);
            g[e] += (CEN && !pl.z_fb) ? v : P.srz * v;
        }
    }
    if (T_ON) {
        T xm[VEC], xp[VEC], wm[VEC], wp[VEC], xm2[VEC], xp2[VEC], fac[VEC];
        ld_into<T, VEC>(xm, pl.xtm + o);  ld_into<T, VEC>(xp, pl.xtp + o);
        ld_into<T, VEC>(wm, pl.wtm + o);  ld_into<T, VEC>(wp, pl.wtp + o);
        if (CEN) { ld_into<T, VEC>(xm2, pl.xtm2 + o); ld_into<T, VEC>(xp2, pl.xtp2 + o); }
        static_factor<T, VEC>(fac, P, i, j0);
        T wc[VEC];
#pragma unroll
        for (int e = 0; e < VEC; ++e) wc[e] = wr[e + 1];
        if constexpr (TS) {
            scale_by<T, VEC>(wm, pl.ts_m, o); scale_by<T, VEC>(wc, pl.ts_c, o); scale_by<T, VEC>(wp, pl.ts_p, o);
        }
#pragma unroll
        for (int e = 0; e < VEC; ++e) {
            const T v = strip_g_axis<T, SCHEME>(pl.t_fb, pl.at, pl.bt, CEN ? xm2[e] : T(0), xm[e], xr[e + 2], xp[e], CEN ? xp2[e] : T(0), wm[e], wc[e], wp[e]);
            g[e] += ((CEN && !pl.t_fb) ? v : P.srt * v) * fac[e];
        }
    }
    Pack<T, VEC> pk;
#pragma unroll
    for (int e = 0; e < VEC; ++e) pk.v[e] = g[e] * (P.inv_div * P.inv_div);
    st_pack<T, VEC>(g_plane + o, pk);
}

template <typename T, int VEC, int SCHEME, bool Z_ON, bool T_ON, bool TS = false>
PYTVB_HD void strip_quad_G(T* g_plane, const GradPlane<T>& pl, const Params<T>& P, int i, int j0, int o) {
    strip_quad_G_impl<T, VEC, SCHEME, Z_ON, T_ON, TS && T_ON>(g_plane, pl, P, i, j0, o);
}


template <typename T, int SCHEME>
PYTVB_HD T pair_w(T wk, T wk1) {
    return SCHEME == UPWIND ? wk : (SCHEME == DOWNWIND ? wk1 : wk + wk1);
}

template <typename T>
PYTVB_HD void row_neighbours(T& l, T& r, const T* row_o, T first, T last, bool has_l, bool has_r, int vec, bool wrow, unsigned m,
                             bool need_l, bool need_r) {
#if defined(__CUDA_ARCH__)
    const int lane = threadIdx.x & 31;
    const T sl = need_l ? __shfl_up_sync(m, last, 1) : first, sr = need_r ? __shfl_down_sync(m, first, 1) : last;
    const bool use_l = wrow && lane > 0, use_r = wrow && lane < 31 && has_r;
    l = !need_l ? first : (use_l ? sl : (has_l ? row_o[-1] : first));
    r = !need_r ? last : (use_r ? sr : (has_r ? row_o[vec] : last));
#else
    (void)wrow; (void)m;
    l = (need_l && has_l) ? row_o[-1] : first;
    r = (need_r && has_r) ? row_o[vec] : last;
#endif
}
PYTVB_HD unsigned sweep_lanes() {
#if defined(__CUDA_ARCH__)
    return __activemask();
#else
    return 1u;
#endif
}

template <typename T>
PYTVB_HD void norm_finish(T s, const Params<T>& P, T& nr, T& w, bool& pos) {
    const T rs = fast_rsqrt(s);
    pos = s > T(0);
    nr = pos ? s * rs * P.inv_div : T(0);
    w = pos ? rs * P.div : T(0);
}
#if defined(__CUDA_ARCH__)
template <>
__device__ __forceinline__ void norm_finish<float>(float s, const Params<float>& P, float& nr, float& w, bool& pos) {
    float rs;
    asm("rsqrt.approx.ftz.f32 %0, %1;" : "=f"(rs) : "f"(fmaxf(s, 1.17549435e-38f)));
    pos = s >= 1.17549435e-38f;
    nr = pos ? s * rs * P.inv_div : 0.0f;
    w = pos ? rs * P.div : 0.0f;
}
#endif

#ifndef PYTVB_TVNORM_UNROLL
#define PYTVB_TVNORM_UNROLL 64
#endif
template <typename T, int VEC, int SCHEME, bool Z_ON, bool T_ON, int R, bool TS, bool FAC>
PYTVB_HD T strip_rows_tv_norm_impl(T* w_plane, T* n_plane, const DualPlane<T>& pl, const Params<T>& P, int i0, int j0) {
    static_assert(SCHEME != CENTRAL, "row-marching sweeps are for the one-sided and hybrid schemes");
    typedef Comp<SCHEME, Z_ON, T_ON> C;
    constexpr bool FWD = C::NEED_FWD, BWD = C::NEED_BWD;
    const int Nj = P.Nj, Ni = P.Ni;
    int o = i0 * Nj + j0;
    T xc[VEC], db[VEC];
    ld_into<T, VEC>(xc, pl.c + o);
    if (BWD) {
        T up[VEC];
        ld_into<T, VEC>(up, pl.c + (i0 > 0 ? o - Nj : o));
#pragma unroll
        for (int e = 0; e < VEC; ++e) db[e] = xc[e] - up[e];
    }
    const bool has_l = j0 > 0, has_r = j0 + VEC < Nj;
    const T rz2 = P.srz * P.srz, rt2 = P.srt * P.srt;
    T sum = T(0);
    constexpr int UNR = PYTVB_TVNORM_UNROLL;
#pragma unroll(UNR)
    for (int r = 0; r < R; ++r) {
        const int i = i0 + r;
        const bool live = r == 0 || i < Ni;
        const int on = i < Ni - 1 ? o + Nj : o;
        T xn[VEC], df[VEC], s[VEC];
        if (FWD || r + 1 < R) {
            ld_into<T, VEC>(xn, pl.c + on);
#pragma unroll
            for (int e = 0; e < VEC; ++e) df[e] = xn[e] - xc[e];
        }
        const T cl = (BWD && has_l) ? pl.c[o - 1] : xc[0], cr = (FWD && has_r) ? pl.c[o + VEC] : xc[VEC - 1];
        if (FWD) {
#pragma unroll
            for (int e = 0; e < VEC; ++e) {
                const T jf = (e + 1 < VEC ? xc[e + 1 < VEC ? e + 1 : e] : cr) - xc[e];
                s[e] = df[e] * df[e];
                s[e] += jf * jf;
            }
        }
        if (BWD) {
#pragma unroll
            for (int e = 0; e < VEC; ++e) {
                const T jb = xc[e] - (e > 0 ? xc[e > 0 ? e - 1 : 0] : cl);
                if (FWD) s[e] += db[e] * db[e]; else s[e] = db[e] * db[e];
                s[e] += jb * jb;
            }
        }
        if (Z_ON) {
            T q[VEC];
            if (FWD) {
                T zp[VEC];
                ld_into<T, VEC>(zp, pl.zp + o);
#pragma unroll
                for (int e = 0; e < VEC; ++e) { const T d = zp[e] - xc[e]; q[e] = d * d; }
            }
            if (BWD) {
                T zm[VEC];
                ld_into<T, VEC>(zm, pl.zm + o);
#pragma unroll
                for (int e = 0; e < VEC; ++e) { const T d = xc[e] - zm[e]; if (FWD) q[e] += d * d; else q[e] = d * d; }
            }
#pragma unroll
            for (int e = 0; e < VEC; ++e) s[e] += rz2 * q[e];
        }
        if (T_ON) {
            T q[VEC];
            if (FWD) {
                T tp[VEC];
                ld_into<T, VEC>(tp, pl.tp + o);
#pragma unroll
                for (int e = 0; e < VEC; ++e) { const T d = tp[e] - xc[e]; q[e] = d * d; }
            }
            if (BWD) {
                T tm[VEC];
                ld_into<T, VEC>(tm, pl.tm + o);
#pragma unroll
                for (int e = 0; e < VEC; ++e) { const T d = xc[e] - tm[e]; if (FWD) q[e] += d * d; else q[e] = d * d; }
            }
            if constexpr (FAC) {
                T fac[VEC];
                const int il = i < Ni ? i : Ni - 1;
                if constexpr (TS) time_factor<T, VEC>(fac, P, pl.ts, il, j0, o); else static_factor<T, VEC>(fac, P, il, j0);
#pragma unroll
                for (int e = 0; e < VEC; ++e) { const T wt = P.srt * fac[e]; s[e] += (wt * wt) * q[e]; }
            } else {
#pragma unroll
                for (int e = 0; e < VEC; ++e) s[e] += rt2 * q[e];
            }
        }
        Pack<T, VEC> w, n;
        T rowsum = T(0);
#pragma unroll
        for (int e = 0; e < VEC; ++e) {
            T nr; bool pos;
            norm_finish<T>(s[e], P, nr, w.v[e], pos);
            n.v[e] = pos ? nr : T(INFINITY);
            rowsum += nr;
        }
        if (live) {
            sum += rowsum;
            if (w_plane) st_pack<T, VEC>(w_plane + o, w);
            if (n_plane) st_pack<T, VEC>(n_plane + o, n);
        }
        if (r + 1 < R) {
#pragma unroll
            for (int e = 0; e < VEC; ++e) { if (BWD) db[e] = df[e]; xc[e] = xn[e]; }
            o = on;
        }
    }
    return sum;
}
template <typename T, int VEC, int SCHEME, bool Z_ON, bool T_ON, int R, bool TS = false, bool FAC = true>
PYTVB_HD T strip_rows_tv_norm(T* w_plane, T* n_plane, const DualPlane<T>& pl, const Params<T>& P, int i0, int j0) {
    return strip_rows_tv_norm_impl<T, VEC, SCHEME, Z_ON, T_ON, R, TS && T_ON, (FAC || TS) && T_ON>(w_plane, n_plane, pl, P, i0, j0);
}

#ifndef PYTVB_TVGRAD_UNROLL
#define PYTVB_TVGRAD_UNROLL 1
#endif
template <typename T, int VEC, int SCHEME, bool Z_ON, bool T_ON, int R, bool TS, bool FAC>
PYTVB_HD void strip_rows_G_impl(T* g_plane, const GradPlane<T>& pl, const Params<T>& P, int i0, int j0, bool wrow) {
    const unsigned lanes = sweep_lanes();
    static_assert(SCHEME != CENTRAL, "row-marching sweeps are for the one-sided and hybrid schemes");
    const int Nj = P.Nj, Ni = P.Ni;
    int o = i0 * Nj + j0;
    T xc[VEC], wc[VEC], ti[VEC];
    ld_into<T, VEC>(xc, pl.x + o);
    ld_into<T, VEC>(wc, pl.w + o);
    {
        T xu[VEC], wu[VEC];
        const int ou = i0 > 0 ? o - Nj : o;
        ld_into<T, VEC>(xu, pl.x + ou);
        ld_into<T, VEC>(wu, pl.w + ou);
#pragma unroll
        for (int e = 0; e < VEC; ++e) ti[e] = (xc[e] - xu[e]) * pair_w<T, SCHEME>(wu[e], wc[e]);
    }
    const bool has_l = j0 > 0, has_r = j0 + VEC < Nj;
    const T k2 = P.inv_div * P.inv_div;
    constexpr int UNR = PYTVB_TVGRAD_UNROLL;
#pragma unroll(UNR)
    for (int r = 0; r < R; ++r) {
        const int i = i0 + r;
        const bool live = r == 0 || i < Ni;
        const int on = i < Ni - 1 ? o + Nj : o;
        T xn[VEC], wn[VEC], g[VEC];
        ld_into<T, VEC>(xn, pl.x + on);
        ld_into<T, VEC>(wn, pl.w + on);
#pragma unroll
        for (int e = 0; e < VEC; ++e) {
            const T tn = (xn[e] - xc[e]) * pair_w<T, SCHEME>(wc[e], wn[e]);
            g[e] = ti[e] - tn;
            ti[e] = tn;
        }
        {
            T xl, xr, wl, wr;
            row_neighbours<T>(xl, xr, pl.x + o, xc[0], xc[VEC - 1], has_l, has_r, VEC, wrow, lanes, true, true);
            row_neighbours<T>(wl, wr, pl.w + o, wc[0], wc[VEC - 1], has_l, has_r, VEC, wrow, lanes, true, true);
            T tj = (xc[0] - xl) * pair_w<T, SCHEME>(wl, wc[0]);
#pragma unroll
            for (int e = 0; e < VEC; ++e) {
                const T xe = e + 1 < VEC ? xc[e + 1 < VEC ? e + 1 : e] : xr, we = e + 1 < VEC ? wc[e + 1 < VEC ? e + 1 : e] : wr;
                const T tn = (xe - xc[e]) * pair_w<T, SCHEME>(wc[e], we);
                g[e] += tj - tn;
                tj = tn;
            }
        }
        if (Z_ON) {
            T xm[VEC], xp[VEC], wm[VEC], wp[VEC];
            ld_into<T, VEC>(xm, pl.xzm + o);  ld_into<T, VEC>(xp, pl.xzp + o);
            ld_into<T, VEC>(wm, pl.wzm + o);  ld_into<T, VEC>(wp, pl.wzp + o);
#pragma unroll
            for (int e = 0; e < VEC; ++e) {
                const T v = (xc[e] - xm[e]) * pair_w<T, SCHEME>(wm[e], wc[e]) - (xp[e] - xc[e]) * pair_w<T, SCHEME>(wc[e], wp[e]);
                g[e] += P.srz * v;
            }
        }
        if (T_ON) {
            T xm[VEC], xp[VEC], wm[VEC], wp[VEC], wq[VEC];
            ld_into<T, VEC>(xm, pl.xtm + o);  ld_into<T, VEC>(xp, pl.xtp + o);
            ld_into<T, VEC>(wm, pl.wtm + o);  ld_into<T, VEC>(wp, pl.wtp + o);
#pragma unroll
            for (int e = 0; e < VEC; ++e) wq[e] = wc[e];
            if constexpr (TS) {
                scale_by<T, VEC>(wm, pl.ts_m, o); scale_by<T, VEC>(wq, pl.ts_c, o); scale_by<T, VEC>(wp, pl.ts_p, o);
            }
            T fac[VEC];
            if constexpr (FAC) static_factor<T, VEC>(fac, P, i < Ni ? i : Ni - 1, j0);
#pragma unroll
            for (int e = 0; e < VEC; ++e) {
                const T v = (xc[e] - xm[e]) * pair_w<T, SCHEME>(wm[e], wq[e]) - (xp[e] - xc[e]) * pair_w<T, SCHEME>(wq[e], wp[e]);
                if constexpr (FAC) g[e] += (P.srt * v) * fac[e]; else g[e] += P.srt * v;
            }
        }
        if (live) {
            Pack<T, VEC> pk;
#pragma unroll
            for (int e = 0; e < VEC; ++e) pk.v[e] = g[e] * k2;
            st_pack<T, VEC>(g_plane + o, pk);
        }
        if (r + 1 < R) {
#pragma unroll
            for (int e = 0; e < VEC; ++e) { xc[e] = xn[e]; wc[e] = wn[e]; }
            o = on;
        }
    }
}
template <typename T, int VEC, int SCHEME, bool Z_ON, bool T_ON, int R, bool TS = false, bool FAC = true>
PYTVB_HD void strip_rows_G(T* g_plane, const GradPlane<T>& pl, const Params<T>& P, int i0, int j0, bool wrow = false) {
    strip_rows_G_impl<T, VEC, SCHEME, Z_ON, T_ON, R, TS && T_ON, FAC && T_ON>(g_plane, pl, P, i0, j0, wrow);
}

template <typename T, int VEC, bool Z_ON, bool T_ON, int R, bool TS, bool FAC>
PYTVB_HD T strip_rows_tv_norm_central(T* w_plane, T* n_plane, const DualPlane<T>& pl, const Params<T>& P, int i0, int j0) {
    const int Nj = P.Nj, Ni = P.Ni;
    int o = i0 * Nj + j0;
    T xu[VEC], xc[VEC];
    ld_into<T, VEC>(xc, pl.c + o);
    ld_into<T, VEC>(xu, pl.c + (i0 > 0 ? o - Nj : o));
    const bool has_l = j0 > 0, has_r = j0 + VEC < Nj;
    const T wz = P.srz * pl.fz, wz2 = wz * wz, wtu = P.srt * pl.ft, wt2u = wtu * wtu;
    T sum = T(0);
#pragma unroll
    for (int r = 0; r < R; ++r) {
        const int i = i0 + r;
        const bool live = r == 0 || i < Ni;
        const int on = i < Ni - 1 ? o + Nj : o;
        T xn[VEC], s[VEC];
        ld_into<T, VEC>(xn, pl.c + on);
        const T fi = (i > 0 && i < Ni - 1) ? T(1) : T(0);
        const T cl = has_l ? pl.c[o - 1] : xc[0], cr = has_r ? pl.c[o + VEC] : xc[VEC - 1];
#pragma unroll
        for (int e = 0; e < VEC; ++e) {
            const int j = j0 + e;
            const T fj = (j > 0 && j < Nj - 1) ? T(1) : T(0);
            const T di = fi * (xn[e] - xu[e]);
            const T dj = fj * ((e + 1 < VEC ? xc[e + 1 < VEC ? e + 1 : e] : cr) - (e > 0 ? xc[e > 0 ? e - 1 : 0] : cl));
            s[e] = di * di;
            s[e] += dj * dj;
        }
        if (Z_ON) {
            T zp[VEC], zm[VEC];
            ld_into<T, VEC>(zp, pl.zp + o);
            ld_into<T, VEC>(zm, pl.zm + o);
#pragma unroll
            for (int e = 0; e < VEC; ++e) { const T d = zp[e] - zm[e]; s[e] += wz2 * (d * d); }
        }
        if (T_ON) {
            T tp[VEC], tm[VEC];
            ld_into<T, VEC>(tp, pl.tp + o);
            ld_into<T, VEC>(tm, pl.tm + o);
            if constexpr (FAC) {
                T fac[VEC];
                const int il = i < Ni ? i : Ni - 1;
                if constexpr (TS) time_factor<T, VEC>(fac, P, pl.ts, il, j0, o); else static_factor<T, VEC>(fac, P, il, j0);
#pragma unroll
                for (int e = 0; e < VEC; ++e) { const T d = tp[e] - tm[e], wt = wtu * fac[e]; s[e] += (wt * wt) * (d * d); }
            } else {
#pragma unroll
                for (int e = 0; e < VEC; ++e) { const T d = tp[e] - tm[e]; s[e] += wt2u * (d * d); }
            }
        }
        Pack<T, VEC> w, n;
        T rowsum = T(0);
#pragma unroll
        for (int e = 0; e < VEC; ++e) {
            T nr; bool pos;
            norm_finish<T>(s[e], P, nr, w.v[e], pos);
            n.v[e] = pos ? nr : T(INFINITY);
            rowsum += nr;
        }
        if (live) {
            sum += rowsum;
            if (w_plane) st_pack<T, VEC>(w_plane + o, w);
            if (n_plane) st_pack<T, VEC>(n_plane + o, n);
        }
        if (r + 1 < R) {
#pragma unroll
            for (int e = 0; e < VEC; ++e) { xu[e] = xc[e]; xc[e] = xn[e]; }
            o = on;
        }
    }
    return sum;
}

template <typename T, int VEC, bool Z_ON, bool T_ON, int R, bool TS>
PYTVB_HD void strip_rows_G_central(T* g_plane, const GradPlane<T>& pl, const Params<T>& P, int i0, int j0) {
    const int Nj = P.Nj, Ni = P.Ni;
    const int o0 = i0 * Nj + j0;
    auto row = [&](int m) { return o0 + ((m < 0 ? 0 : (m > Ni - 1 ? Ni - 1 : m)) - i0) * Nj; };
    auto valid = [&](int m) { return m >= 1 && m <= Ni - 2; };
    T xc[VEC], xp[VEC], Cm[VEC], Cc[VEC];
    ld_into<T, VEC>(xc, pl.x + o0);
    ld_into<T, VEC>(xp, pl.x + row(i0 + 1));
    {
        T xm2[VEC], xm1[VEC], wm1[VEC], w0[VEC];
        ld_into<T, VEC>(xm2, pl.x + row(i0 - 2));
        ld_into<T, VEC>(xm1, pl.x + row(i0 - 1));
        ld_into<T, VEC>(wm1, pl.w + row(i0 - 1));
        ld_into<T, VEC>(w0, pl.w + o0);
        const T vm = valid(i0 - 1) ? T(1) : T(0), vc = valid(i0) ? T(1) : T(0);
#pragma unroll
        for (int e = 0; e < VEC; ++e) {
            Cm[e] = vm * ((xc[e] - xm2[e]) * wm1[e]);
            Cc[e] = vc * ((xp[e] - xm1[e]) * w0[e]);
        }
    }
    int o = o0;
    constexpr int UNR = PYTVB_TVGRAD_UNROLL;
#pragma unroll(UNR)
    for (int r = 0; r < R; ++r) {
        const int i = i0 + r;
        if (r == 0 || i < Ni) {
            T x2[VEC], wn[VEC], g[VEC];
            ld_into<T, VEC>(x2, pl.x + row(i + 2));
            ld_into<T, VEC>(wn, pl.w + row(i + 1));
            const T vn = valid(i + 1) ? T(1) : T(0);
#pragma unroll
            for (int e = 0; e < VEC; ++e) {
                const T Cn = vn * ((x2[e] - xc[e]) * wn[e]);
                g[e] = Cm[e] - Cn;
                Cm[e] = Cc[e];
                Cc[e] = Cn;
                xc[e] = xp[e];
                xp[e] = x2[e];
            }
            strip_quad_G_impl<T, VEC, CENTRAL, Z_ON, T_ON, TS && T_ON, false>(g_plane, pl, P, i, j0, o, g);
            o += Nj;
        }
    }
}

}
```

Before: 55.74 billion.

## Precompute in-plane adjoint prefix in dual kernel to cut primal loads

The dual update kernel now also computes the in-plane (row, column, time) part of D^T y while the freshly updated duals are still in registers and shared memory, and writes it to a new per-voxel buffer q. Tile-edge rows and columns are left for the primal kernel. The primal kernel then reads q plus the z-direction dual terms instead of re-reading most dual components, which cuts global memory traffic in the primal pass. The cost is an extra full-size buffer write and read, more shared-memory use in the dual kernel, and a restructured DT computation that must reproduce the same rounding. The new path is used for the ROF variant with full-precision duals and M <= 8.

```diff
diff --git a/__graft_entry__.py b/__graft_entry__.py
--- a/__graft_entry__.py
+++ b/__graft_entry__.py
@@ -7,8 +7,8 @@
 CSRC = os.path.join(ROOT, "pytv-4d_b200", "csrc")
 ARCH = ["-gencode", "arch=compute_100a,code=sm_100a"]
 NVCC_FLAGS = ARCH + ["-lineinfo", "-O3", "-std=c++17", "-Xcompiler", "-fPIC"]
-SOURCES = ["api.cu", "ops.cu", "tv.cu", "tv_tile.cu", "tv_tile_f64.cu", "tv_tile_norms.cu", "tv_tile_norms_f64.cu", "cp.cu", "cp_extra.cu", "cp_data.cu", "host_api.cu"]
-HEADERS = ["core.cuh", "strip_core.cuh", "tile_core.cuh", "tile2_core.cuh", "kernels.cuh", "kernels2.cuh", "kernels_tile.cuh", "tv_path.cuh", "tv_args.cuh", "tmap.cuh", "tv_tile_impl.cuh", "host_common.cuh", os.path.join("..", "..", "include", "pytv_b200.h")]
+SOURCES = ["api.cu", "ops.cu", "tv.cu", "tv_tile.cu", "tv_tile_f64.cu", "tv_tile_norms.cu", "tv_tile_norms_f64.cu", "cp.cu", "cp_extra.cu", "cp_data.cu", "cp_adj.cu", "host_api.cu"]
+HEADERS = ["core.cuh", "strip_core.cuh", "adj_core.cuh", "tile_core.cuh", "tile2_core.cuh", "kernels.cuh", "kernels2.cuh", "kernels_tile.cuh", "tv_path.cuh", "tv_args.cuh", "tmap.cuh", "tv_tile_impl.cuh", "host_common.cuh", os.path.join("..", "..", "include", "pytv_b200.h")]
 
 
 def source_hash():
diff --git a/include/pytv_b200.h b/include/pytv_b200.h
--- a/include/pytv_b200.h
+++ b/include/pytv_b200.h
@@ -77,6 +77,17 @@
                          const void* x0, double tau, double theta, double* d_fid_or_null, const void* halo_lo, const void* halo_hi,
                          void* mirror_prev, void* mirror_next, void* ws, void* stream);
 
+int pytvb_cp_dual_adj(const pytvb_problem* pb, const void* xbar, void* y, void* q, double lam, double sigma, double* d_l21_or_null,
+                      const void* halo_lo, const void* halo_hi, void* ws, void* stream);
+int pytvb_cp_dual_adj_p2p(const pytvb_problem* pb, const void* xbar, void* y, void* q, double lam, double sigma, double* d_l21_or_null,
+                          const void* halo_lo, const void* halo_hi, void* mirror_prev, void* mirror_next, void* ws, void* stream);
+int pytvb_cp_primal_adj(const pytvb_problem* pb, int data_term, const void* data_weight, const void* y, const void* q, void* x, void* xbar,
+                        const void* x0, double tau, double theta, double* d_fid_or_null, const void* halo_lo, const void* halo_hi, void* ws,
+                        void* stream);
+int pytvb_cp_primal_adj_p2p(const pytvb_problem* pb, int data_term, const void* data_weight, const void* y, const void* q, void* x, void* xbar,
+                            const void* x0, double tau, double theta, double* d_fid_or_null, const void* halo_lo, const void* halo_hi,
+                            void* mirror_prev, void* mirror_next, void* ws, void* stream);
+
 int pytvb_cp_dual_f16y(const pytvb_problem* pb, const void* xbar, void* y_half, double lam, double sigma, double* d_l21_or_null,
                        const void* halo_lo, const void* halo_hi, void* ws, void* stream);
 int pytvb_cp_primal_rof_f16y(const pytvb_problem* pb, const void* y_half, void* x, void* xbar, const void* x0, double lam, double tau,
diff --git a/pytv-4d_b200/_lib.py b/pytv-4d_b200/_lib.py
--- a/pytv-4d_b200/_lib.py
+++ b/pytv-4d_b200/_lib.py
@@ -62,6 +62,12 @@
     "pytvb_cp_primal_p2p": (ctypes.c_int, [_PB, ctypes.c_int, _VP, _VP, _VP, _VP, ctypes.c_double, ctypes.c_double, _VP, _VP, _VP, _VP, _VP, _VP, _VP]),
     "pytvb_cp_primal_data": (ctypes.c_int, [_PB, ctypes.c_int, _VP, _VP, _VP, _VP, _VP, ctypes.c_double, ctypes.c_double, _VP, _VP, _VP, _VP, _VP, _VP,
                                             _VP]),
+    "pytvb_cp_dual_adj": (ctypes.c_int, [_PB, _VP, _VP, _VP, ctypes.c_double, ctypes.c_double, _VP, _VP, _VP, _VP, _VP]),
+    "pytvb_cp_dual_adj_p2p": (ctypes.c_int, [_PB, _VP, _VP, _VP, ctypes.c_double, ctypes.c_double, _VP, _VP, _VP, _VP, _VP, _VP, _VP]),
+    "pytvb_cp_primal_adj": (ctypes.c_int, [_PB, ctypes.c_int, _VP, _VP, _VP, _VP, _VP, _VP, ctypes.c_double, ctypes.c_double, _VP, _VP, _VP, _VP,
+                                           _VP]),
+    "pytvb_cp_primal_adj_p2p": (ctypes.c_int, [_PB, ctypes.c_int, _VP, _VP, _VP, _VP, _VP, _VP, ctypes.c_double, ctypes.c_double, _VP, _VP, _VP,
+                                               _VP, _VP, _VP, _VP]),
     "pytvb_cp_dual_f16y": (ctypes.c_int, [_PB, _VP, _VP, ctypes.c_double, ctypes.c_double, _VP, _VP, _VP, _VP, _VP]),
     "pytvb_cp_primal_rof_f16y": (ctypes.c_int, [_PB, _VP, _VP, _VP, _VP, ctypes.c_double, ctypes.c_double, ctypes.c_double, _VP, _VP, _VP, _VP, _VP]),
     "pytvb_tv_host": (ctypes.c_int, [_PB, _VP, _VP, _VP, ctypes.POINTER(ctypes.c_double)]),
diff --git a/pytv-4d_b200/cp.py b/pytv-4d_b200/cp.py
--- a/pytv-4d_b200/cp.py
+++ b/pytv-4d_b200/cp.py
@@ -66,6 +66,15 @@
         _lib.check(self.lib.pytvb_cp_primal_p2p(ctypes.byref(pb), 0 if variant == "rof" else 1, _dev.ptr(y), _dev.ptr(x), _dev.ptr(aux), _dev.ptr(x0),
                                                 tau, c2, _dev.ptr(d_fid), _dev.ptr(lo), _dev.ptr(hi), mirror_prev, mirror_next, _dev.ptr(ws),
                                                 _dev.stream_ptr()))
+
+    def cp_dual_adj(self, pb, xbar, y, q, lam, sigma, d_l21, lo, hi, mirror_prev, mirror_next, ws):
+        _lib.check(self.lib.pytvb_cp_dual_adj_p2p(ctypes.byref(pb), _dev.ptr(xbar), _dev.ptr(y), _dev.ptr(q), lam, sigma, _dev.ptr(d_l21), _dev.ptr(lo),
+                                                  _dev.ptr(hi), mirror_prev, mirror_next, _dev.ptr(ws), _dev.stream_ptr()))
+
+    def cp_primal_adj(self, pb, data_term, w, y, q, x, xbar, x0, tau, theta, d_fid, lo, hi, mirror_prev, mirror_next, ws):
+        _lib.check(self.lib.pytvb_cp_primal_adj_p2p(ctypes.byref(pb), DATA_TERMS[data_term], _dev.ptr(w), _dev.ptr(y), _dev.ptr(q), _dev.ptr(x),
+                                                    _dev.ptr(xbar), _dev.ptr(x0), tau, theta, _dev.ptr(d_fid), _dev.ptr(lo), _dev.ptr(hi), mirror_prev,
+                                                    mirror_next, _dev.ptr(ws), _dev.stream_ptr()))
 
     def workspace(self, pb, device):
         return _dev.reduce_workspace(pb, device)
@@ -261,6 +270,8 @@
         if self._data and (variant != "rof" or self.dual_dtype != dt):
             raise ValueError("data_term='l1' and data_weight need variant='rof' and full-precision duals")
         self.y = torch.zeros((shape[0], self.Nd) + shape[1:], dtype=self.dual_dtype, device=dev)
+        self._adj = isinstance(self.ops, CudaOps) and variant == "rof" and self.dual_dtype == dt and shape[1] <= 8
+        self.q = torch.empty_like(self.x0) if self._adj else None
         self.scal = torch.zeros(6, dtype=torch.float64, device=dev)
         self.overlap = os.environ.get("PYTVB_OVERLAP", "0") == "1"
         self._pending = None
@@ -345,6 +356,9 @@
         lo = u[a - 1] if a > 0 else self._img_lo
         hi = u[b] if b < Nz else self._img_hi
         d = self.scal[slot:slot + 1] if self.track_energy else None
+        if self._adj:
+            self.ops.cp_dual_adj(self._sub_problem(a, b), u[a:b], self.y[a:b], self.q[a:b], self.lam, self.sigma, d, lo, hi, None, None, self.ws)
+            return
         self.ops.cp_dual(self._sub_problem(a, b), u[a:b], self.y[a:b], self.lam, self.sigma, d, lo, hi, self.ws)
 
     def _primal_range(self, a, b, slot):
@@ -354,6 +368,10 @@
         lo = self.y[a - 1, self._zf] if a > 0 else self._fld_lo
         hi = self.y[b, self._zb] if b < Nz else self._fld_hi
         d = self.scal[3 + slot:4 + slot] if self.track_energy else None
+        if self._adj:
+            self.ops.cp_primal_adj(self._sub_problem(a, b), self.data_term, self._dw[a:b] if self._dw is not None else None, self.y[a:b], self.q[a:b],
+                                   self.x[a:b], self.aux[a:b], self.x0[a:b], self.tau, self.theta, d, lo, hi, None, None, self.ws)
+            return
         if self._data:
             self.ops.cp_primal_data(self._sub_problem(a, b), self.data_term, self._dw[a:b] if self._dw is not None else None, self.y[a:b], self.x[a:b],
                                     self.aux[a:b], self.x0[a:b], self.tau, self.theta, d, lo, hi, None, None, self.ws)
@@ -387,8 +405,12 @@
                 self._peer.barrier()
             self._pending = ()
             d = self.scal[0:1] if self.track_energy else None
-            self.ops.cp_dual_p2p(self.pb, self._dual_input(), self.y, self.lam, self.sigma, d, self._img_lo, self._img_hi, self._mir_A[0],
-                                 self._mir_A[1], self.ws)
+            if self._adj:
+                self.ops.cp_dual_adj(self.pb, self._dual_input(), self.y, self.q, self.lam, self.sigma, d, self._img_lo, self._img_hi, self._mir_A[0],
+                                     self._mir_A[1], self.ws)
+            else:
+                self.ops.cp_dual_p2p(self.pb, self._dual_input(), self.y, self.lam, self.sigma, d, self._img_lo, self._img_hi, self._mir_A[0],
+                                     self._mir_A[1], self.ws)
             self._peer.barrier()
             self._field_req = ()
             return
@@ -412,7 +434,10 @@
             self.scal[3:6].zero_()
         if self._peer is not None:
             d = self.scal[3:4] if self.track_energy else None
-            if self._data:
+            if self._adj:
+                self.ops.cp_primal_adj(self.pb, self.data_term, self._dw, self.y, self.q, self.x, self.aux, self.x0, self.tau, self.theta, d,
+                                       self._fld_lo, self._fld_hi, self._mir_B[0], self._mir_B[1], self.ws)
+            elif self._data:
                 self.ops.cp_primal_data(self.pb, self.data_term, self._dw, self.y, self.x, self.aux, self.x0, self.tau, self.theta, d, self._fld_lo,
                                         self._fld_hi, self._mir_B[0], self._mir_B[1], self.ws)
             else:
@@ -453,7 +478,7 @@
 
     def _graph_state_key(self):
         return (self.x0.data_ptr(), self.x.data_ptr(), self.aux.data_ptr(), self.y.data_ptr(), self.lam, self.sigma, self.tau, self.theta, self.sigma_A,
-                self._dw.data_ptr() if self._dw is not None else 0)
+                self._dw.data_ptr() if self._dw is not None else 0, self.q.data_ptr() if self.q is not None else 0)
 
     def step(self, n=1):
         g = getattr(self, "_graph", None)
diff --git a/pytv-4d_b200/csrc/adj_core.cuh b/pytv-4d_b200/csrc/adj_core.cuh
--- /dev/null
+++ b/pytv-4d_b200/csrc/adj_core.cuh
@@ -0,0 +1,215 @@
+#pragma once
+#include "strip_core.cuh"
+
+#ifndef PYTVB_STRIP_R
+#define PYTVB_STRIP_R 4
+#endif
+#ifndef PYTVB_ADJ_R
+#define PYTVB_ADJ_R 32
+#endif
+
+namespace pytvb {
+
+constexpr int ADJ_R = PYTVB_ADJ_R;
+constexpr int ADJ_MAXM = 8;
+constexpr int ADJ_THREADS = 256;
+static_assert(ADJ_R % PYTVB_STRIP_R == 0, "the L21 partial sums follow the row groups of cp_dual_strip_kernel");
+
+PYTVB_HD int adj_tile_quads(int M) { return M == 1 ? 256 : (M == 2 ? 128 : (M <= 4 ? 64 : 32)); }
+
+PYTVB_HD bool adj_edge_row(int i, int Ni) { return (i % ADJ_R == 0 && i > 0) || (i % ADJ_R == ADJ_R - 1 && i < Ni - 1); }
+PYTVB_HD bool adj_edge_col(int tq, int TWq, int j0, int vec, int Nj) { return (tq == 0 && j0 > 0) || (tq == TWq - 1 && j0 + vec < Nj); }
+
+template <int VEC> struct AdjSlots { static constexpr int value = 3 + 2 * VEC; };
+template <typename T, int VEC>
+struct AdjShared {
+    T* b;
+    PYTVB_HD T& jf0(int k) const { return b[k]; }
+    PYTVB_HD T& jf1(int k) const { return b[ADJ_THREADS + k]; }
+    PYTVB_HD T& jb0(int k) const { return b[2 * ADJ_THREADS + k]; }
+    PYTVB_HD T& tf(int e, int k) const { return b[(3 + e) * ADJ_THREADS + k]; }
+    PYTVB_HD T& tb(int e, int k) const { return b[(3 + VEC + e) * ADJ_THREADS + k]; }
+};
+
+template <typename T, int VEC, int SCHEME, bool Z_ON, bool T_ON>
+struct AdjThread {
+    static constexpr int ND = Comp<SCHEME, Z_ON, T_ON>::ND;
+    DualPlane<T, T> pl;
+    MirrorPlanes<T> mir;
+    T* qp;
+    int t, tq, j0, TWq;
+    bool act, cedge;
+    T at, bt;
+    T yv[ND][VEC], tsc[VEC];
+    T cIFm[VEC], cIF[VEC], cIB[VEC], cCol[VEC], cT[VEC];
+    T g;
+    double l21;
+};
+
+template <typename T, int VEC, int SCHEME, bool Z_ON, bool T_ON, bool MIR>
+PYTVB_HD void adj_thread_init(AdjThread<T, VEC, SCHEME, Z_ON, T_ON>& s, const ImgView<T>& Xb, T* y, T* qd, const Params<T>& P, const MirrorBufs<T>& mb,
+                              int z, int cb, int tid, int TWq, int W) {
+    s.TWq = TWq;
+    s.t = tid / TWq;
+    s.tq = tid - s.t * TWq;
+    const int qj = cb * TWq + s.tq;
+    s.j0 = qj * VEC;
+    s.act = s.t < P.M && qj < W;
+    const int tc = s.t < P.M ? s.t : P.M - 1;
+    s.pl = make_dual_plane<T, SCHEME, T>(Xb, y, P, z, tc);
+    s.mir = MirrorPlanes<T>{nullptr, nullptr};
+    if constexpr (MIR) s.mir = mirror_planes<T>(mb, P, z, tc);
+    s.qp = qd + (long long)z * P.sZ + (long long)tc * P.sT;
+    s.cedge = adj_edge_col(s.tq, TWq, s.j0, VEC, P.Nj);
+    s.at = s.bt = T(0);
+    if (T_ON) {
+        adj_factors<T, SCHEME>(s.at, s.bt, tc, P.M, P.t_fwd_fallback != 0);
+        s.at *= P.srt;
+        s.bt *= P.srt;
+    }
+#pragma unroll
+    for (int e = 0; e < VEC; ++e) s.cIFm[e] = s.cIF[e] = s.cIB[e] = s.cCol[e] = s.cT[e] = T(0);
+    s.g = T(0);
+    s.l21 = 0.0;
+}
+
+template <typename T, int VEC, int SCHEME, bool Z_ON, bool T_ON>
+PYTVB_HD void adj_finish_row(AdjThread<T, VEC, SCHEME, Z_ON, T_ON>& s, const Params<T>& P, int k, const T* ib_next) {
+    constexpr bool NF = (SCHEME != DOWNWIND), NB = (SCHEME != UPWIND), CTR = (SCHEME == CENTRAL);
+    T a, b;
+    adj_factors<T, SCHEME>(a, b, k, P.Ni, false);
+    Pack<T, VEC> pk;
+#pragma unroll
+    for (int e = 0; e < VEC; ++e) {
+        const T f_m = NF ? (k > 0 ? s.cIFm[e] : s.cIF[e]) : T(0);
+        const T f_c = (!CTR && NF) ? s.cIF[e] : T(0);
+        const T b_c = (!CTR && NB) ? s.cIB[e] : T(0);
+        const T b_p = NB ? ib_next[e] : T(0);
+        const T rows = adj_term<T, SCHEME>(a, b, f_m, f_c, b_c, b_p, false);
+        pk.v[e] = s.cedge ? adj_rows_t<T, T_ON>(rows, s.cT[e]) : adj_prefix<T, T_ON>(rows, s.cCol[e], s.cT[e]);
+    }
+    if (!adj_edge_row(k, P.Ni)) st_pack<T, VEC>(s.qp + k * P.Nj + s.j0, pk);
+}
+
+template <typename T, int VEC, int SCHEME, bool Z_ON, bool T_ON>
+PYTVB_HD void adj_prefetch_next(const AdjThread<T, VEC, SCHEME, Z_ON, T_ON>& s, const Params<T>& P, int i) {
+#if defined(__CUDA_ARCH__)
+    const int Nj = P.Nj, o = i * Nj + s.j0;
+#pragma unroll
+    for (int k = 0; k < Comp<SCHEME, Z_ON, T_ON>::ND; ++k) asm volatile("prefetch.global.L2 [%0];" ::"l"(s.pl.y + (long long)k * P.sC + o + Nj));
+    asm volatile("prefetch.global.L2 [%0];" ::"l"(s.pl.c + (i + 2 < P.Ni ? o + 2 * Nj : o + Nj)));
+#else
+    (void)s; (void)P; (void)i;
+#endif
+}
+
+template <typename T, int VEC, int SCHEME, bool Z_ON, bool T_ON, bool TS, bool MIR>
+PYTVB_HD void adj_row_update(AdjThread<T, VEC, SCHEME, Z_ON, T_ON>& s, const Params<T>& P, int i, const AdjShared<T, VEC>& sh, int tid, T sig, T lam) {
+    typedef Comp<SCHEME, Z_ON, T_ON> C;
+    if (!s.act) return;
+    const int Nj = P.Nj, o = i * Nj + s.j0;
+    s.g += strip_quad_cp_dual_y<T, VEC, SCHEME, Z_ON, T_ON, T, TS, MIR>(s.yv, s.pl, P, i, s.j0, o, i > 0 ? o - Nj : o, i < P.Ni - 1 ? o + Nj : o, sig,
+                                                                       lam, s.mir);
+    if (i % PYTVB_STRIP_R == PYTVB_STRIP_R - 1 || i == P.Ni - 1) {
+        s.l21 += (double)s.g * (double)P.inv_div;
+        s.g = T(0);
+    }
+    sh.jf0(tid) = s.yv[C::J_F][0];
+    sh.jf1(tid) = s.yv[C::J_F][VEC - 1];
+    sh.jb0(tid) = s.yv[C::J_B][0];
+    if (T_ON) {
+#pragma unroll
+        for (int e = 0; e < VEC; ++e) s.tsc[e] = T(1);
+        if constexpr (TS) {
+            const Pack<T, VEC> sc = ld_pack<T, VEC>(s.pl.ts + o);
+#pragma unroll
+            for (int e = 0; e < VEC; ++e) s.tsc[e] = sc.v[e];
+        }
+#pragma unroll
+        for (int e = 0; e < VEC; ++e) {
+            sh.tf(e, tid) = TS ? mul_rn(s.yv[C::T_F][e], s.tsc[e]) : s.yv[C::T_F][e];
+            sh.tb(e, tid) = TS ? mul_rn(s.yv[C::T_B][e], s.tsc[e]) : s.yv[C::T_B][e];
+        }
+    }
+}
+
+template <typename T, int VEC, int SCHEME, bool Z_ON, bool T_ON, bool TS>
+PYTVB_HD void adj_row_finish(AdjThread<T, VEC, SCHEME, Z_ON, T_ON>& s, const Params<T>& P, int i, bool first, const AdjShared<T, VEC>& sh, int tid) {
+    typedef Comp<SCHEME, Z_ON, T_ON> C;
+    constexpr bool NF = (SCHEME != DOWNWIND), NB = (SCHEME != UPWIND), CTR = (SCHEME == CENTRAL);
+    constexpr bool HB = (SCHEME == HYBRID || SCHEME == DOWNWIND);
+    if (!s.act) return;
+    const int Nj = P.Nj, TWq = s.TWq;
+    T col[VEC], tt[VEC];
+    {
+        T jb[VEC];
+#pragma unroll
+        for (int e = 0; e < VEC; ++e) jb[e] = (SCHEME == HYBRID) ? s.yv[C::J_B][e] : T(0);
+        const bool has_l = s.j0 > 0 && s.tq > 0, has_r = s.j0 + VEC < Nj && s.tq < TWq - 1;
+        const T jf_l = (NF && has_l) ? sh.jf1(tid - 1) : T(0);
+        const T jf_r = (CTR && has_r) ? sh.jf0(tid + 1) : T(0);
+        const T jb_r = (HB && has_r) ? sh.jb0(tid + 1) : T(0);
+        adj_cols<T, VEC, SCHEME>(col, s.yv[C::J_F], jb, jf_l, jf_r, jb_r, s.j0, Nj);
+    }
+    if (T_ON) {
+        const bool tfb = P.t_fwd_fallback != 0, up_form = !CTR || tfb;
+        T ifs[VEC], f_m[VEC], f_c[VEC], b_c[VEC], b_p[VEC], fac[VEC];
+#pragma unroll
+        for (int e = 0; e < VEC; ++e) {
+            ifs[e] = TS ? mul_rn(s.yv[C::I_F][e], s.tsc[e]) : s.yv[C::I_F][e];
+            f_m[e] = NF ? (s.t > 0 ? sh.tf(e, tid - TWq) : ifs[e]) : T(0);
+            f_c[e] = (up_form && NF) ? sh.tf(e, tid) : T(0);
+            b_c[e] = (!CTR && NB) ? sh.tb(e, tid) : T(0);
+            b_p[e] = (NB && !(CTR && tfb)) ? (s.t < P.M - 1 ? sh.tb(e, tid + TWq) : ifs[e]) : T(0);
+        }
+        static_factor<T, VEC>(fac, P, i, s.j0);
+        adj_time<T, VEC, SCHEME>(tt, f_m, f_c, b_c, b_p, fac, s.at, s.bt, tfb);
+    } else {
+        zero_into<T, VEC>(tt);
+    }
+    if (!first) adj_finish_row(s, P, i - 1, s.yv[C::I_B]);
+#pragma unroll
+    for (int e = 0; e < VEC; ++e) {
+        s.cIFm[e] = s.cIF[e];
+        s.cIF[e] = s.yv[C::I_F][e];
+        s.cIB[e] = s.yv[C::I_B][e];
+        s.cCol[e] = col[e];
+        s.cT[e] = tt[e];
+    }
+}
+
+template <typename T, int VEC, int SCHEME, bool Z_ON, bool T_ON>
+PYTVB_HD void adj_tile_end(AdjThread<T, VEC, SCHEME, Z_ON, T_ON>& s, const Params<T>& P, int i_end) {
+    if (s.act && i_end == P.Ni) adj_finish_row(s, P, P.Ni - 1, s.cIB);
+}
+
+template <typename T, int VEC, int SCHEME, bool Z_ON, bool T_ON, int VARIANT, bool WM, bool TS, bool MIR>
+PYTVB_HD T adj_quad_primal(const PrimalPlane<T, T>& pl, const T* qd, T* x, T* xbar, const T* x0, const T* w, const Params<T>& P, int i, int j0,
+                           bool cedge, T tau, T c1, T theta, T tau_x0, MirrorPlanes<T> mir) {
+    typedef Comp<SCHEME, Z_ON, T_ON> C;
+    constexpr bool NF = (SCHEME != DOWNWIND), CTR = (SCHEME == CENTRAL), HB = (SCHEME == HYBRID || SCHEME == DOWNWIND);
+    const int o = i * P.Nj + j0;
+    T dty[VEC];
+    if (adj_edge_row(i, P.Ni)) {
+        strip_quad_DT<T, VEC, SCHEME, Z_ON, T_ON, false, T, TS>(dty, pl, P, i, j0, o, i > 0 ? o - P.Nj : o, i < P.Ni - 1 ? o + P.Nj : o);
+    } else {
+        const T* qo = qd + pl.img + o;
+        const T* yJ_F = pl.y + (long long)C::J_F * P.sC + o;
+        const T* yJ_B = pl.y + (long long)C::J_B * P.sC + o;
+        const bool l = cedge && NF && j0 > 0, rf = cedge && CTR && j0 + VEC < P.Nj, rb = cedge && HB && j0 + VEC < P.Nj;
+        T jf[VEC], jb[VEC];
+        ld_into<T, VEC>(jf, cedge ? yJ_F : qo);
+        if (SCHEME == HYBRID) ld_into<T, VEC>(jb, cedge ? yJ_B : qo); else zero_into<T, VEC>(jb);
+        T jf_l = *(l ? yJ_F - 1 : qo), jf_r = *(rf ? yJ_F + VEC : qo), jb_r = *(rb ? yJ_B + VEC : qo);
+        jf_l = l ? jf_l : T(0); jf_r = rf ? jf_r : T(0); jb_r = rb ? jb_r : T(0);
+        const Pack<T, VEC> pre = ld_pack<T, VEC>(qo);
+        T zt[VEC], cols[VEC];
+        if (Z_ON) strip_quad_DT_z<T, VEC, SCHEME, Z_ON, T_ON, false, T>(zt, pl, P, o); else zero_into<T, VEC>(zt);
+        adj_cols<T, VEC, SCHEME>(cols, jf, jb, jf_l, jf_r, jb_r, j0, P.Nj);
+#pragma unroll
+        for (int e = 0; e < VEC; ++e) dty[e] = adj_finish<T, Z_ON>(cedge ? add_rn(pre.v[e], cols[e]) : pre.v[e], zt[e], P.inv_div);
+    }
+    return cp_primal_update<T, VEC, Z_ON, VARIANT, MIR, WM>(dty, x, xbar, x0, pl.img + o, o, tau, c1, theta, tau_x0, mir, w);
+}
+
+}
diff --git a/pytv-4d_b200/csrc/cp_adj.cu b/pytv-4d_b200/csrc/cp_adj.cu
--- /dev/null
+++ b/pytv-4d_b200/csrc/cp_adj.cu
@@ -0,0 +1,235 @@
+#include <stdlib.h>
+
+#include "host_common.cuh"
+#include "kernels2.cuh"
+#include "adj_core.cuh"
+
+using namespace pytvb;
+
+namespace pytvb {
+
+static_assert(ADJ_THREADS == CTA_THREADS, "an A' tile is one CTA");
+
+struct AdjTiling {
+    int TWq, W, ncb, nz;
+    FastDiv d_ncb, d_nz;
+    long long nblocks;
+};
+inline AdjTiling make_adj_tiling(int Nj, int Ni, int M, int nz, int vec) {
+    AdjTiling t;
+    t.TWq = adj_tile_quads(M);
+    t.W = (Nj + vec - 1) / vec;
+    t.ncb = (t.W + t.TWq - 1) / t.TWq;
+    t.nz = nz;
+    t.d_ncb = make_fastdiv((unsigned)t.ncb);
+    t.d_nz = make_fastdiv((unsigned)nz);
+    t.nblocks = (long long)t.ncb * nz * ((Ni + ADJ_R - 1) / ADJ_R);
+    return t;
+}
+
+template <typename T, int VEC, int SCHEME, bool Z_ON, bool T_ON, bool TS, bool MIR>
+__global__ void __launch_bounds__(CTA_THREADS, PYTVB_DUAL_MINB) cp_dual_adj_kernel(ImgView<T> Xb, T* __restrict__ y, T* __restrict__ qd,
+                                                                                  double* __restrict__ partial, Params<T> P, T sig, T lam,
+                                                                                  AdjTiling tl, MirrorBufs<T> mb) {
+    __shared__ T sm[2][AdjSlots<T_ON ? VEC : 0>::value * CTA_THREADS];
+    unsigned b = blockIdx.x, cb, zi;
+    tl.d_ncb.divmod(b, b, cb);
+    tl.d_nz.divmod(b, b, zi);
+    const int i0 = (int)b * ADJ_R, nrows = min(ADJ_R, P.Ni - i0), tid = threadIdx.x;
+    AdjThread<T, VEC, SCHEME, Z_ON, T_ON> s;
+    adj_thread_init<T, VEC, SCHEME, Z_ON, T_ON, MIR>(s, Xb, y, qd, P, mb, (int)zi, (int)cb, tid, tl.TWq, tl.W);
+    for (int r = 0; r < nrows; ++r) {
+        const int bf = r & 1;
+        const AdjShared<T, VEC> sh{sm[bf]};
+        if (s.act && r + 1 < nrows) adj_prefetch_next(s, P, i0 + r);
+        adj_row_update<T, VEC, SCHEME, Z_ON, T_ON, TS, MIR>(s, P, i0 + r, sh, tid, sig, lam);
+        __syncthreads();
+        adj_row_finish<T, VEC, SCHEME, Z_ON, T_ON, TS>(s, P, i0 + r, r == 0, sh, tid);
+    }
+    adj_tile_end(s, P, i0 + nrows);
+    if (partial) {
+        const double bs = block_sum(s.l21);
+        store_or_finish(bs, partial, P);
+    }
+}
+
+template <typename T, int VEC, int SCHEME, bool Z_ON, bool T_ON, int VARIANT, bool WM, int R, bool TS, bool MIR>
+__global__ void __launch_bounds__(CTA_THREADS, PYTVB_PRIMAL_MINB) cp_primal_adj_kernel(FieldView<T> Y, const T* __restrict__ qd, T* __restrict__ x,
+                                                                                      T* __restrict__ xbar, const T* __restrict__ x0,
+                                                                                      const T* __restrict__ w, double* __restrict__ partial,
+                                                                                      Params<T> P, T tau, T c1, T theta, T tau_x0, Tiling tl,
+                                                                                      int twq, MirrorBufs<T> mb) {
+    const QuadIdx q = decode_quad(tl, (P.Ni + R - 1) / R, VEC);
+    T fid = T(0);
+    if (q.active) {
+        const PrimalPlane<T, T> pl = make_primal_plane<T, SCHEME, Z_ON, T_ON, T>(Y, P, q.z, q.t);
+        MirrorPlanes<T> mir{nullptr, nullptr};
+        if constexpr (MIR) mir = mirror_planes<T>(mb, P, q.z, q.t);
+        const bool cedge = adj_edge_col((q.j0 / VEC) & (twq - 1), twq, q.j0, VEC, P.Nj);
+        const int i0 = q.i * R;
+#pragma unroll
+        for (int r = 0; r < R; ++r) {
+            const int i = i0 + r;
+            if (i < P.Ni)
+                fid += adj_quad_primal<T, VEC, SCHEME, Z_ON, T_ON, VARIANT, WM, TS, MIR>(pl, qd, x, xbar, x0, w, P, i, q.j0, cedge, tau, c1, theta, tau_x0,
+                                                                                         mir);
+        }
+    }
+    if (partial) {
+        const double bs = block_sum((double)fid);
+        store_or_finish(bs, partial, P);
+    }
+}
+
+}
+
+namespace {
+
+template <typename T> struct AdjDualArgs { ImgView<T> Xb; T* y; T* q; double* partial; Params<T> P; T sig, lam; cudaStream_t st; long long* nb; T* mir_prev; T* mir_next; };
+
+template <typename T, int VEC, int SCHEME, bool Z, bool TT> struct LaunchDualAdj {
+    static int run(const AdjDualArgs<T>& a) {
+        const AdjTiling tl = make_adj_tiling(a.P.Nj, a.P.Ni, a.P.M, a.P.Nz, VEC);
+        PYTVB_REQUIRE(tl.nblocks > 0 && tl.nblocks < 2147483647LL, "grid of %lld CTAs is out of range", tl.nblocks);
+        const bool ts = TT && a.P.tscale, mir = Z && (a.mir_prev || a.mir_next);
+        const MirrorBufs<T> mb{a.mir_prev, a.mir_next};
+        const unsigned nb = (unsigned)tl.nblocks;
+        if (ts && mir) cp_dual_adj_kernel<T, VEC, SCHEME, Z, TT, TT, Z><<<nb, CTA_THREADS, 0, a.st>>>(a.Xb, a.y, a.q, a.partial, a.P, a.sig, a.lam, tl, mb);
+        else if (ts) cp_dual_adj_kernel<T, VEC, SCHEME, Z, TT, TT, false><<<nb, CTA_THREADS, 0, a.st>>>(a.Xb, a.y, a.q, a.partial, a.P, a.sig, a.lam, tl, mb);
+        else if (mir) cp_dual_adj_kernel<T, VEC, SCHEME, Z, TT, false, Z><<<nb, CTA_THREADS, 0, a.st>>>(a.Xb, a.y, a.q, a.partial, a.P, a.sig, a.lam, tl, mb);
+        else cp_dual_adj_kernel<T, VEC, SCHEME, Z, TT, false, false><<<nb, CTA_THREADS, 0, a.st>>>(a.Xb, a.y, a.q, a.partial, a.P, a.sig, a.lam, tl, mb);
+        count_launches(1);
+        PYTVB_CUDA(cudaGetLastError());
+        *a.nb = tl.nblocks;
+        return PYTVB_OK;
+    }
+};
+
+template <typename T> struct AdjPrimalArgs {
+    FieldView<T> Y; const T* q; T* x; T* xbar; const T* x0; const T* w; double* partial; Params<T> P; T tau, theta; int term; cudaStream_t st;
+    long long* nb; T* mir_prev; T* mir_next;
+};
+
+template <typename T, int VEC, int SCHEME, bool Z, bool TT, int VARIANT, bool WM>
+void launch_primal_adj(const AdjPrimalArgs<T>& a, const Tiling& tl) {
+    constexpr int R = PYTVB_STRIP_R;
+    const bool ts = TT && a.P.tscale, mir = Z && (a.mir_prev || a.mir_next);
+    const MirrorBufs<T> mb{a.mir_prev, a.mir_next};
+    const unsigned nb = (unsigned)tl.nblocks;
+    const T c1 = VARIANT == 0 ? T(1) / (T(1) + a.tau) : T(0), tx = VARIANT == 0 ? T(-1) : a.tau;
+    const int twq = adj_tile_quads(a.P.M);
+#define PYTVB_ADJ_B(TSV, MIRV)                                                                                                                  \
+    cp_primal_adj_kernel<T, VEC, SCHEME, Z, TT, VARIANT, WM, R, TSV, MIRV><<<nb, CTA_THREADS, 0, a.st>>>(a.Y, a.q, a.x, a.xbar, a.x0, a.w, a.partial, \
+                                                                                                      a.P, a.tau, c1, a.theta, tx, tl, twq, mb)
+    if (ts && mir) PYTVB_ADJ_B(TT, Z);
+    else if (ts) PYTVB_ADJ_B(TT, false);
+    else if (mir) PYTVB_ADJ_B(false, Z);
+    else PYTVB_ADJ_B(false, false);
+#undef PYTVB_ADJ_B
+}
+
+template <typename T, int VEC, int SCHEME, bool Z, bool TT> struct LaunchPrimalAdj {
+    static int run(const AdjPrimalArgs<T>& a) {
+        const Tiling tl = make_strip_tiling<PYTVB_STRIP_R>(a.P.Nj, a.P.Ni, a.P.M, a.P.Nz, VEC);
+        if (int rc = check_grid(tl)) return rc;
+        if (a.term == PYTVB_DATA_L2 && !a.w) launch_primal_adj<T, VEC, SCHEME, Z, TT, 0, false>(a, tl);
+        else if (a.term == PYTVB_DATA_L2) launch_primal_adj<T, VEC, SCHEME, Z, TT, 2, true>(a, tl);
+        else if (a.w) launch_primal_adj<T, VEC, SCHEME, Z, TT, 3, true>(a, tl);
+        else launch_primal_adj<T, VEC, SCHEME, Z, TT, 3, false>(a, tl);
+        count_launches(1);
+        PYTVB_CUDA(cudaGetLastError());
+        *a.nb = tl.nblocks;
+        return PYTVB_OK;
+    }
+};
+
+template <typename T>
+int run_dual_adj(const pytvb_problem* pb, const void* xbar, void* y, void* q, double lam, double sigma, double* d_l21, const void* lo, const void* hi,
+                 void* mir_prev, void* mir_next, void* ws, cudaStream_t st) {
+    const Axes ax = axes_of(pb);
+    AdjDualArgs<T> a;
+    a.Xb = ImgView<T>{(const T*)xbar, (const T*)lo, (const T*)hi, 1};
+    a.y = (T*)y;
+    a.q = (T*)q;
+    a.partial = d_l21 ? reduce_partials(ws) : nullptr;
+    a.P = make_params<T>(pb);
+    arm_reduction(a.P, ws, d_l21);
+    a.sig = (T)sigma * a.P.inv_div;
+    a.lam = (T)lam;
+    a.mir_prev = (T*)mir_prev; a.mir_next = (T*)mir_next;
+    a.st = st;
+    long long nb = 0;
+    a.nb = &nb;
+    const int vec = pick_vec<T>(pb, {xbar, y, q, lo, hi, mir_prev, mir_next});
+    if (int rc = dispatch<LaunchDualAdj, T>(vec, pb->scheme, ax.z_on, ax.t_on, a)) return rc;
+    return d_l21 ? finish_reduction(a.partial, nb, d_l21, st) : PYTVB_OK;
+}
+
+template <typename T>
+int run_primal_adj(const pytvb_problem* pb, int term, const void* w, const void* y, const void* q, void* x, void* xbar, const void* x0, double tau,
+                   double theta, double* d_fid, const void* lo, const void* hi, void* mir_prev, void* mir_next, void* ws, cudaStream_t st) {
+    const Axes ax = axes_of(pb);
+    AdjPrimalArgs<T> a;
+    a.Y = FieldView<T>{(const T*)y, (const T*)lo, (const T*)hi};
+    a.q = (const T*)q;
+    a.x = (T*)x; a.xbar = (T*)xbar; a.x0 = (const T*)x0; a.w = (const T*)w;
+    a.partial = d_fid ? reduce_partials(ws) : nullptr;
+    a.P = make_params<T>(pb);
+    arm_reduction(a.P, ws, d_fid);
+    a.tau = (T)tau; a.theta = (T)theta;
+    a.term = term;
+    a.mir_prev = (T*)mir_prev; a.mir_next = (T*)mir_next;
+    a.st = st;
+    long long nb = 0;
+    a.nb = &nb;
+    const int vec = pick_vec<T>(pb, {y, q, x, xbar, x0, w, lo, hi, mir_prev, mir_next});
+    if (int rc = dispatch<LaunchPrimalAdj, T>(vec, pb->scheme, ax.z_on, ax.t_on, a)) return rc;
+    return d_fid ? finish_reduction(a.partial, nb, d_fid, st) : PYTVB_OK;
+}
+
+}
+
+extern "C" {
+
+int pytvb_cp_dual_adj_p2p(const pytvb_problem* pb, const void* xbar, void* y, void* q, double lam, double sigma, double* d_l21_or_null,
+                          const void* halo_lo, const void* halo_hi, void* mirror_prev, void* mirror_next, void* ws, void* stream) {
+    if (int rc = check_problem(pb)) return rc;
+    PYTVB_REQUIRE(xbar && y && q, "xbar, y and q must not be NULL");
+    PYTVB_REQUIRE(pb->M <= ADJ_MAXM, "M = %lld: the dual pass with the adjoint prefix spans at most %d frames", (long long)pb->M, ADJ_MAXM);
+    PYTVB_REQUIRE(!d_l21_or_null || ws, "a reduction workspace is required when d_l21 is requested");
+    PYTVB_REQUIRE(lam >= 0, "lam must be >= 0");
+    if (int rc = check_halos(pb, axes_of(pb).z_on, false, halo_lo, halo_hi)) return rc;
+    cudaStream_t st = (cudaStream_t)stream;
+    return pb->dtype == PYTVB_F32 ? run_dual_adj<float>(pb, xbar, y, q, lam, sigma, d_l21_or_null, halo_lo, halo_hi, mirror_prev, mirror_next, ws, st)
+                                  : run_dual_adj<double>(pb, xbar, y, q, lam, sigma, d_l21_or_null, halo_lo, halo_hi, mirror_prev, mirror_next, ws, st);
+}
+
+int pytvb_cp_dual_adj(const pytvb_problem* pb, const void* xbar, void* y, void* q, double lam, double sigma, double* d_l21_or_null, const void* halo_lo,
+                      const void* halo_hi, void* ws, void* stream) {
+    return pytvb_cp_dual_adj_p2p(pb, xbar, y, q, lam, sigma, d_l21_or_null, halo_lo, halo_hi, nullptr, nullptr, ws, stream);
+}
+
+int pytvb_cp_primal_adj_p2p(const pytvb_problem* pb, int data_term, const void* data_weight, const void* y, const void* q, void* x, void* xbar,
+                            const void* x0, double tau, double theta, double* d_fid_or_null, const void* halo_lo, const void* halo_hi,
+                            void* mirror_prev, void* mirror_next, void* ws, void* stream) {
+    if (int rc = check_problem(pb)) return rc;
+    PYTVB_REQUIRE(data_term == PYTVB_DATA_L2 || data_term == PYTVB_DATA_L1, "data_term must be PYTVB_DATA_L2 (0) or PYTVB_DATA_L1 (1)");
+    PYTVB_REQUIRE(y && q && x && xbar && x0, "y, q, x, xbar and x0 must not be NULL");
+    PYTVB_REQUIRE(pb->M <= ADJ_MAXM, "M = %lld: the dual pass with the adjoint prefix spans at most %d frames", (long long)pb->M, ADJ_MAXM);
+    PYTVB_REQUIRE(!d_fid_or_null || ws, "a reduction workspace is required when d_fid is requested");
+    if (int rc = check_halos(pb, axes_of(pb).z_on, true, halo_lo, halo_hi)) return rc;
+    cudaStream_t st = (cudaStream_t)stream;
+    return pb->dtype == PYTVB_F32 ? run_primal_adj<float>(pb, data_term, data_weight, y, q, x, xbar, x0, tau, theta, d_fid_or_null, halo_lo, halo_hi,
+                                                          mirror_prev, mirror_next, ws, st)
+                                  : run_primal_adj<double>(pb, data_term, data_weight, y, q, x, xbar, x0, tau, theta, d_fid_or_null, halo_lo, halo_hi,
+                                                           mirror_prev, mirror_next, ws, st);
+}
+
+int pytvb_cp_primal_adj(const pytvb_problem* pb, int data_term, const void* data_weight, const void* y, const void* q, void* x, void* xbar,
+                        const void* x0, double tau, double theta, double* d_fid_or_null, const void* halo_lo, const void* halo_hi, void* ws,
+                        void* stream) {
+    return pytvb_cp_primal_adj_p2p(pb, data_term, data_weight, y, q, x, xbar, x0, tau, theta, d_fid_or_null, halo_lo, halo_hi, nullptr, nullptr, ws,
+                                   stream);
+}
+
+}
diff --git a/pytv-4d_b200/csrc/strip_core.cuh b/pytv-4d_b200/csrc/strip_core.cuh
--- a/pytv-4d_b200/csrc/strip_core.cuh
+++ b/pytv-4d_b200/csrc/strip_core.cuh
@@ -165,12 +165,12 @@
     r.next = (m.next && z == P.Nz - 1) ? m.next + (long long)t * P.sT : nullptr;
     return r;
 }
-template <typename T, int VEC, int SCHEME, bool Z_ON, bool T_ON, typename YT = T, bool TS = false, bool MIR = false>
-PYTVB_HD T strip_quad_cp_dual(const DualPlane<T, YT>& pl, const Params<T>& P, int i, int j0, int o, int o_up, int o_dn, T sig, T lam,
-                              MirrorPlanes<YT> mir = MirrorPlanes<YT>{nullptr, nullptr}) {
+template <typename T, int VEC, int SCHEME, bool Z_ON, bool T_ON, typename YT, bool TS, bool MIR>
+PYTVB_HD T strip_quad_cp_dual_y(T (*y)[VEC], const DualPlane<T, YT>& pl, const Params<T>& P, int i, int j0, int o, int o_up, int o_dn, T sig, T lam,
+                                MirrorPlanes<YT> mir) {
     typedef Comp<SCHEME, Z_ON, T_ON> C;
     constexpr int ND = C::ND;
-    T y[ND][VEC], d[ND][VEC];
+    T d[ND][VEC];
 #pragma unroll
     for (int k = 0; k < ND; ++k) ld_y<T, YT, VEC>(y[k], pl.y + (long long)k * P.sC + o);
     strip_raw_diffs<T, VEC, SCHEME, Z_ON, T_ON, YT, TS>(d, pl, P, i, j0, o, o_up, o_dn);
@@ -191,13 +191,18 @@
         for (int k = 0; k < ND; ++k) y[k][e] *= scale;
     }
 #pragma unroll
-#pragma unroll
     for (int k = 0; k < ND; ++k) st_y<T, YT, VEC>(pl.y + (long long)k * P.sC + o, y[k]);
     if constexpr (MIR && Z_ON) {
         if (mir.prev) st_y<T, YT, VEC>(mir.prev + o, y[C::Z_B]);
         if (mir.next) st_y<T, YT, VEC>(mir.next + o, y[C::Z_F]);
     }
     return l21;
+}
+template <typename T, int VEC, int SCHEME, bool Z_ON, bool T_ON, typename YT = T, bool TS = false, bool MIR = false>
+PYTVB_HD T strip_quad_cp_dual(const DualPlane<T, YT>& pl, const Params<T>& P, int i, int j0, int o, int o_up, int o_dn, T sig, T lam,
+                              MirrorPlanes<YT> mir = MirrorPlanes<YT>{nullptr, nullptr}) {
+    T y[Comp<SCHEME, Z_ON, T_ON>::ND][VEC];
+    return strip_quad_cp_dual_y<T, VEC, SCHEME, Z_ON, T_ON, YT, TS, MIR>(y, pl, P, i, j0, o, o_up, o_dn, sig, lam, mir);
 }
 
 template <typename T, int VEC, int SCHEME, bool Z_ON, bool T_ON, bool TS = false>
@@ -294,12 +299,93 @@
     return p;
 }
 
+PYTVB_HD float add_rn(float a, float b) {
+#if defined(__CUDA_ARCH__)
+    return __fadd_rn(a, b);
+#else
+    return a + b;
+#endif
+}
+PYTVB_HD float sub_rn(float a, float b) {
+#if defined(__CUDA_ARCH__)
+    return __fsub_rn(a, b);
+#else
+    return a - b;
+#endif
+}
+PYTVB_HD float mul_rn(float a, float b) {
+#if defined(__CUDA_ARCH__)
+    return __fmul_rn(a, b);
+#else
+    return a * b;
+#endif
+}
+PYTVB_HD double add_rn(double a, double b) {
+#if defined(__CUDA_ARCH__)
+    return __dadd_rn(a, b);
+#else
+    return a + b;
+#endif
+}
+PYTVB_HD double sub_rn(double a, double b) {
+#if defined(__CUDA_ARCH__)
+    return __dsub_rn(a, b);
+#else
+    return a - b;
+#endif
+}
+PYTVB_HD double mul_rn(double a, double b) {
+#if defined(__CUDA_ARCH__)
+    return __dmul_rn(a, b);
+#else
+    return a * b;
+#endif
+}
+
 template <typename T, int SCHEME>
-PYTVB_HD void adj_operands(T& m, T& p, T f_m, T f_c, T b_c, T b_p, bool fallback) {
+PYTVB_HD T adj_term(T a, T b, T f_m, T f_c, T b_c, T b_p, bool fallback) {
+    T m, p;
     if (SCHEME == UPWIND || (SCHEME == CENTRAL && fallback)) { m = f_m; p = f_c; }
     else if (SCHEME == DOWNWIND) { m = b_c; p = b_p; }
-    else if (SCHEME == HYBRID) { m = f_m + b_c; p = f_c + b_p; }
+    else if (SCHEME == HYBRID) { m = add_rn(f_m, b_c); p = add_rn(f_c, b_p); }
     else { m = f_m; p = b_p; }
+    return sub_rn(mul_rn(a, m), mul_rn(b, p));
+}
+
+template <typename T, int VEC, int SCHEME>
+PYTVB_HD void adj_cols(T* out, const T* jf, const T* jb, T jf_left, T jf_right, T jb_right, int j0, int Nj) {
+    T f[VEC + 2], bq[VEC + 2];
+    f[0] = jf_left;
+#pragma unroll
+    for (int e = 0; e < VEC; ++e) f[e + 1] = jf[e];
+    f[VEC + 1] = jf_right;
+#pragma unroll
+    for (int e = 0; e < VEC + 2; ++e) bq[e] = (SCHEME == DOWNWIND) ? f[e] : T(0);
+    if (SCHEME == HYBRID) {
+#pragma unroll
+        for (int e = 0; e < VEC; ++e) bq[e + 1] = jb[e];
+    }
+    if (SCHEME == HYBRID || SCHEME == DOWNWIND) bq[VEC + 1] = jb_right;
+#pragma unroll
+    for (int e = 0; e < VEC; ++e) {
+        T a, b;
+        adj_factors<T, SCHEME>(a, b, j0 + e, Nj, false);
+        out[e] = (SCHEME == CENTRAL) ? adj_term<T, SCHEME>(a, b, f[e], T(0), T(0), f[e + 2], false)
+                                     : adj_term<T, SCHEME>(a, b, f[e], f[e + 1], bq[e + 1], bq[e + 2], false);
+    }
+}
+
+template <typename T, bool T_ON>
+PYTVB_HD T adj_rows_t(T rows, T t) {
+    return T_ON ? add_rn(rows, t) : rows;
+}
+template <typename T, bool T_ON>
+PYTVB_HD T adj_prefix(T rows, T cols, T t) {
+    return add_rn(adj_rows_t<T, T_ON>(rows, t), cols);
+}
+template <typename T, bool Z_ON>
+PYTVB_HD T adj_finish(T prefix, T z, T inv_div) {
+    return mul_rn(Z_ON ? add_rn(prefix, z) : prefix, inv_div);
 }
 
 template <typename T, int VEC> struct CgLoad;
@@ -326,8 +412,23 @@
     return v;
 }
 
+template <typename T, int VEC>
+PYTVB_HD void scale_by_rn(T* v, const T* ts_plane, int o) {
+    if (ts_plane) {
+        const Pack<T, VEC> sc = ld_pack<T, VEC>(ts_plane + o);
+#pragma unroll
+        for (int e = 0; e < VEC; ++e) v[e] = mul_rn(v[e], sc.v[e]);
+    }
+}
+
+template <typename T, int VEC, int SCHEME>
+PYTVB_HD void adj_time(T* out, const T* f_m, const T* f_c, const T* b_c, const T* b_p, const T* fac, T at, T bt, bool fb) {
+#pragma unroll
+    for (int e = 0; e < VEC; ++e) out[e] = mul_rn(adj_term<T, SCHEME>(at, bt, f_m[e], f_c[e], b_c[e], b_p[e], fb), fac[e]);
+}
+
 template <typename T, int VEC, int SCHEME, bool Z_ON, bool T_ON, bool CG, typename YT, bool TS>
-PYTVB_HD void strip_quad_DT_impl(T* out, const PrimalPlane<T, YT>& pl, const Params<T>& P, int i, int j0, int o, int o_up, int o_dn) {
+PYTVB_HD void strip_quad_DT_prefix(T* pre, const PrimalPlane<T, YT>& pl, const Params<T>& P, int i, int j0, int o, int o_up, int o_dn) {
     typedef Comp<SCHEME, Z_ON, T_ON> C;
     constexpr bool NF = (SCHEME != DOWNWIND);
     constexpr bool NB = (SCHEME != UPWIND);
@@ -336,7 +437,7 @@
     const YT* yI_B = pl.y + (long long)C::I_B * P.sC;
     const YT* yJ_F = pl.y + (long long)C::J_F * P.sC;
     const YT* yJ_B = pl.y + (long long)C::J_B * P.sC;
-    T acc[VEC];
+    T rows[VEC], cols[VEC], tt[VEC];
     {
         T a, b, f_m[VEC], f_c[VEC], b_c[VEC], b_p[VEC];
         adj_factors<T, SCHEME>(a, b, i, P.Ni, false);
@@ -345,51 +446,16 @@
         if (!CTR && NB) ld_field<T, VEC, CG>(b_c, yI_B + o); else zero_into<T, VEC>(b_c);
         if (NB) ld_field<T, VEC, CG>(b_p, yI_B + o_dn); else zero_into<T, VEC>(b_p);
 #pragma unroll
-        for (int e = 0; e < VEC; ++e) {
-            T m, p;
-            adj_operands<T, SCHEME>(m, p, f_m[e], f_c[e], b_c[e], b_p[e], false);
-            acc[e] = a * m - b * p;
-        }
+        for (int e = 0; e < VEC; ++e) rows[e] = adj_term<T, SCHEME>(a, b, f_m[e], f_c[e], b_c[e], b_p[e], false);
     }
     {
-        T f[VEC + 2], bq[VEC + 2];
-#pragma unroll
-        for (int e = 0; e < VEC + 2; ++e) bq[e] = T(0);
-        ld_field<T, VEC, CG>(f + 1, yJ_F + o);
-        f[0] = (NF && j0 > 0) ? ld_field1<T, CG>(yJ_F + o - 1) : T(0);
-        f[VEC + 1] = (CTR && j0 + VEC < P.Nj) ? ld_field1<T, CG>(yJ_F + o + VEC) : T(0);
-        if (SCHEME == HYBRID || SCHEME == DOWNWIND) {
-            if (SCHEME == HYBRID) ld_field<T, VEC, CG>(bq + 1, yJ_B + o);
-            else {
-#pragma unroll
-                for (int e = 0; e < VEC + 2; ++e) bq[e] = f[e];
-            }
-            bq[VEC + 1] = (j0 + VEC < P.Nj) ? ld_field1<T, CG>(yJ_B + o + VEC) : T(0);
-        }
-#pragma unroll
-        for (int e = 0; e < VEC; ++e) {
-            const int j = j0 + e;
-            T a, b, m, p;
-            adj_factors<T, SCHEME>(a, b, j, P.Nj, false);
-            if (CTR) adj_operands<T, SCHEME>(m, p, f[e], T(0), T(0), f[e + 2], false);
-            else adj_operands<T, SCHEME>(m, p, f[e], f[e + 1], bq[e + 1], bq[e + 2], false);
-            acc[e] += a * m - b * p;
-        }
-    }
-    if (Z_ON) {
-        const bool fb = P.z_fwd_fallback != 0;
-        const bool up_form = !CTR || fb;
-        T f_m[VEC], f_c[VEC], b_c[VEC], b_p[VEC];
-        if (NF) ld_field<T, VEC, CG>(f_m, pl.zf_m + o); else zero_into<T, VEC>(f_m);
-        if (up_form && NF) ld_field<T, VEC, CG>(f_c, pl.y + (long long)C::Z_F * P.sC + o); else zero_into<T, VEC>(f_c);
-        if (!CTR && NB) ld_field<T, VEC, CG>(b_c, pl.y + (long long)C::Z_B * P.sC + o); else zero_into<T, VEC>(b_c);
-        if (NB && !(CTR && fb)) ld_field<T, VEC, CG>(b_p, pl.zb_p + o); else zero_into<T, VEC>(b_p);
-#pragma unroll
-        for (int e = 0; e < VEC; ++e) {
-            T m, p;
-            adj_operands<T, SCHEME>(m, p, f_m[e], f_c[e], b_c[e], b_p[e], fb);
-            acc[e] += pl.az * m - pl.bz * p;
-        }
+        T jf[VEC], jb[VEC];
+        ld_field<T, VEC, CG>(jf, yJ_F + o);
+        if (SCHEME == HYBRID) ld_field<T, VEC, CG>(jb, yJ_B + o); else zero_into<T, VEC>(jb);
+        const T jf_l = (NF && j0 > 0) ? ld_field1<T, CG>(yJ_F + o - 1) : T(0);
+        const T jf_r = (CTR && j0 + VEC < P.Nj) ? ld_field1<T, CG>(yJ_F + o + VEC) : T(0);
+        const T jb_r = ((SCHEME == HYBRID || SCHEME == DOWNWIND) && j0 + VEC < P.Nj) ? ld_field1<T, CG>(yJ_B + o + VEC) : T(0);
+        adj_cols<T, VEC, SCHEME>(cols, jf, jb, jf_l, jf_r, jb_r, j0, P.Nj);
     }
     if (T_ON) {
         const bool fb = P.t_fwd_fallback != 0;
@@ -400,19 +466,38 @@
         if (!CTR && NB) ld_field<T, VEC, CG>(b_c, pl.y + (long long)C::T_B * P.sC + o); else zero_into<T, VEC>(b_c);
         if (NB && !(CTR && fb)) ld_field<T, VEC, CG>(b_p, pl.tb_p + o); else zero_into<T, VEC>(b_p);
         if constexpr (TS) {
-            scale_by<T, VEC>(f_m, pl.ts_m, o); scale_by<T, VEC>(f_c, pl.ts_c, o);
-            scale_by<T, VEC>(b_c, pl.ts_c, o); scale_by<T, VEC>(b_p, pl.ts_p, o);
+            scale_by_rn<T, VEC>(f_m, pl.ts_m, o); scale_by_rn<T, VEC>(f_c, pl.ts_c, o);
+            scale_by_rn<T, VEC>(b_c, pl.ts_c, o); scale_by_rn<T, VEC>(b_p, pl.ts_p, o);
         }
         static_factor<T, VEC>(fac, P, i, j0);
-#pragma unroll
-        for (int e = 0; e < VEC; ++e) {
-            T m, p;
-            adj_operands<T, SCHEME>(m, p, f_m[e], f_c[e], b_c[e], b_p[e], fb);
-            acc[e] += (pl.at * m - pl.bt * p) * fac[e];
-        }
-    }
-#pragma unroll
-    for (int e = 0; e < VEC; ++e) out[e] = acc[e] * P.inv_div;
+        adj_time<T, VEC, SCHEME>(tt, f_m, f_c, b_c, b_p, fac, pl.at, pl.bt, fb);
+    }
+#pragma unroll
+    for (int e = 0; e < VEC; ++e) pre[e] = adj_prefix<T, T_ON>(rows[e], cols[e], T_ON ? tt[e] : T(0));
+}
+
+template <typename T, int VEC, int SCHEME, bool Z_ON, bool T_ON, bool CG, typename YT>
+PYTVB_HD void strip_quad_DT_z(T* zt, const PrimalPlane<T, YT>& pl, const Params<T>& P, int o) {
+    typedef Comp<SCHEME, Z_ON, T_ON> C;
+    constexpr bool NF = (SCHEME != DOWNWIND), NB = (SCHEME != UPWIND), CTR = (SCHEME == CENTRAL);
+    const bool fb = P.z_fwd_fallback != 0;
+    const bool up_form = !CTR || fb;
+    T f_m[VEC], f_c[VEC], b_c[VEC], b_p[VEC];
+    if (NF) ld_field<T, VEC, CG>(f_m, pl.zf_m + o); else zero_into<T, VEC>(f_m);
+    if (up_form && NF) ld_field<T, VEC, CG>(f_c, pl.y + (long long)C::Z_F * P.sC + o); else zero_into<T, VEC>(f_c);
+    if (!CTR && NB) ld_field<T, VEC, CG>(b_c, pl.y + (long long)C::Z_B * P.sC + o); else zero_into<T, VEC>(b_c);
+    if (NB && !(CTR && fb)) ld_field<T, VEC, CG>(b_p, pl.zb_p + o); else zero_into<T, VEC>(b_p);
+#pragma unroll
+    for (int e = 0; e < VEC; ++e) zt[e] = adj_term<T, SCHEME>(pl.az, pl.bz, f_m[e], f_c[e], b_c[e], b_p[e], fb);
+}
+
+template <typename T, int VEC, int SCHEME, bool Z_ON, bool T_ON, bool CG, typename YT, bool TS>
+PYTVB_HD void strip_quad_DT_impl(T* out, const PrimalPlane<T, YT>& pl, const Params<T>& P, int i, int j0, int o, int o_up, int o_dn) {
+    T pre[VEC], zt[VEC];
+    strip_quad_DT_prefix<T, VEC, SCHEME, Z_ON, T_ON, CG, YT, TS>(pre, pl, P, i, j0, o, o_up, o_dn);
+    if (Z_ON) strip_quad_DT_z<T, VEC, SCHEME, Z_ON, T_ON, CG, YT>(zt, pl, P, o); else zero_into<T, VEC>(zt);
+#pragma unroll
+    for (int e = 0; e < VEC; ++e) out[e] = adj_finish<T, Z_ON>(pre[e], zt[e], P.inv_div);
 }
 
 template <typename T, int VEC, int SCHEME, bool Z_ON, bool T_ON, bool CG = false, typename YT = T, bool TS = false>
@@ -420,14 +505,10 @@
     strip_quad_DT_impl<T, VEC, SCHEME, Z_ON, T_ON, CG, YT, TS && T_ON>(out, pl, P, i, j0, o, o_up, o_dn);
 }
 
-template <typename T, int VEC, int SCHEME, bool Z_ON, bool T_ON, int VARIANT, bool CG = false, typename YT = T, bool TS = false, bool MIR = false,
-          bool WM = false>
-PYTVB_HD T strip_quad_cp_primal(T* x, T* aux, const T* x0, const PrimalPlane<T, YT>& pl, const Params<T>& P, int i, int j0, int o, int o_up, int o_dn,
-                                T tau, T c1, T c2, T tau_x0 = T(-1), MirrorPlanes<T> mir = MirrorPlanes<T>{nullptr, nullptr}, const T* wgt = nullptr) {
-    T dty[VEC];
-    strip_quad_DT<T, VEC, SCHEME, Z_ON, T_ON, CG, YT, TS>(dty, pl, P, i, j0, o, o_up, o_dn);
+template <typename T, int VEC, bool Z_ON, int VARIANT, bool MIR, bool WM>
+PYTVB_HD T cp_primal_update(const T* dty, T* x, T* aux, const T* x0, long long off, int o, T tau, T c1, T c2, T tau_x0, MirrorPlanes<T> mir,
+                            const T* wgt) {
     if (tau_x0 < T(0)) tau_x0 = tau;
-    const long long off = pl.img + o;
     const Pack<T, VEC> xo = ld_pack<T, VEC>(x + off), x0q = ld_pack<T, VEC>(x0 + off);
     Pack<T, VEC> xn, ax;
     T fid = T(0);
@@ -481,6 +562,15 @@
         if (mir.next) st_pack<T, VEC>(mir.next + o, u);
     }
     return fid;
+}
+
+template <typename T, int VEC, int SCHEME, bool Z_ON, bool T_ON, int VARIANT, bool CG = false, typename YT = T, bool TS = false, bool MIR = false,
+          bool WM = false>
+PYTVB_HD T strip_quad_cp_primal(T* x, T* aux, const T* x0, const PrimalPlane<T, YT>& pl, const Params<T>& P, int i, int j0, int o, int o_up, int o_dn,
+                                T tau, T c1, T c2, T tau_x0 = T(-1), MirrorPlanes<T> mir = MirrorPlanes<T>{nullptr, nullptr}, const T* wgt = nullptr) {
+    T dty[VEC];
+    strip_quad_DT<T, VEC, SCHEME, Z_ON, T_ON, CG, YT, TS>(dty, pl, P, i, j0, o, o_up, o_dn);
+    return cp_primal_update<T, VEC, Z_ON, VARIANT, MIR, WM>(dty, x, aux, x0, pl.img + o, o, tau, c1, c2, tau_x0, mir, wgt);
 }
 
 template <typename T>
```

Measured after the change: 60.26 billion (median of 6 runs). 8.1% higher.
